# Nelarius/rayfinder

Hardware: AMD Instinct MI355X
Metric: Mrays/sec at 1920x1080 Sponza, 8 bounces; achieved HBM GB/s on traversal (higher is better)
Workload: dtype f32

## Files before the change

include/rayfinder_amd.h:

```cpp
#ifndef RAYFINDER_AMD_H
#define RAYFINDER_AMD_H

#include <stddef.h>
#include <stdint.h>

#ifdef __cplusplus
extern "C" {
#endif

#define RF_API __attribute__((visibility("default")))

typedef enum rf_status
{
    RF_OK = 0,
    RF_ERROR_INVALID_ARGUMENT = 1,
    RF_ERROR_RUNTIME = 2,
    RF_ERROR_NO_DEVICE = 3,
    RF_ERROR_OUT_OF_RANGE = 4,
} rf_status;

RF_API const char* rf_last_error_message(void);
RF_API const char* rf_version(void);

typedef struct rf_camera
// ... 92 lines not shown
{
    uint32_t iterations;
    float    sigma_color, sigma_normal, sigma_depth;
} rf_denoise_parameters;
RF_API int rf_denoise_default_parameters(rf_denoise_parameters* out);
RF_API int rf_renderer_denoise(rf_renderer* r, const rf_denoise_parameters* params);
RF_API int rf_renderer_read_denoised(rf_renderer* r, float* rgba, uint32_t* bgra8, uint32_t* sample_count);
RF_API int rf_denoise_images(int32_t device_ordinal, uint32_t width, uint32_t height, uint32_t samples, const float* color_sum4, const float* albedo_coverage4,
                             const float* normal_depth4, const rf_denoise_parameters* params, float exposure, float* out_rgba, uint32_t* out_bgra8);
RF_API int rf_denoise_tiles(int32_t device_ordinal, uint32_t width, uint32_t height, const uint32_t* tile_samples, const float* color_sum4,
                            const float* albedo_coverage4, const float* normal_depth4, const rf_denoise_parameters* params, float exposure, float* out_rgba,
                            uint32_t* out_bgra8);

RF_API int rf_renderer_set_direct(rf_renderer* r, int enabled);
RF_API int rf_renderer_read_direct(rf_renderer* r, float* direct_sum4, uint32_t* direct_sample_count);
RF_API int rf_denoise_split_default_parameters(rf_denoise_parameters* direct, rf_denoise_parameters* indirect);
RF_API int rf_renderer_denoise_split(rf_renderer* r, const rf_denoise_parameters* direct, const rf_denoise_parameters* indirect);
RF_API int rf_denoise_split_images(int32_t device_ordinal, uint32_t width, uint32_t height, uint32_t samples, const float* color_sum4, const float* direct_sum4,
                                   const float* albedo_coverage4, const float* normal_depth4, const rf_denoise_parameters* direct, const rf_denoise_parameters* indirect,
                                   float exposure, float* out_rgba, uint32_t* out_bgra8);

typedef struct rf_noise_estimate
{
    double   mean_error;
    float    max_error;
    uint32_t worst_tile, samples;
    uint64_t pixels, nonfinite_pixels;
} rf_noise_estimate;
RF_API int rf_renderer_set_moments(rf_renderer* r, int enabled);
RF_API int rf_renderer_read_moments(rf_renderer* r, float* sumsq4, uint32_t* moment_sample_count);
RF_API int rf_renderer_noise_estimate(rf_renderer* r, rf_noise_estimate* out, float* error_map, float* tile_sum, float* tile_max);
RF_API int rf_noise_estimate_images(int32_t device_ordinal, uint32_t width, uint32_t height, uint32_t samples, const float* color_sum4, const float* sumsq4,
                                    rf_noise_estimate* out, float* error_map, float* tile_sum, float* tile_max);
RF_API int rf_renderer_render_until(rf_renderer* r, float target_mean_error, uint32_t check_every, uint32_t max_frames, uint32_t* frames_rendered,
                                    rf_noise_estimate* last);

#define RF_BUCKETS_TILE_COUNTS 0x100u
#define RF_BUCKETS_SHARD_TILE_COUNTS 0x400u
RF_API int rf_renderer_set_buckets(rf_renderer* r, uint32_t K);
RF_API int rf_renderer_read_buckets(rf_renderer* r, float* buckets, uint32_t* K, uint32_t* bucket_sample_count);
RF_API int rf_renderer_robust_mean(rf_renderer* r);
RF_API int rf_renderer_read_robust_mean(rf_renderer* r, float* rgba, uint32_t* bgra8, uint8_t* trim, uint32_t* sample_count);
RF_API int rf_robust_mean_images(int32_t device_ordinal, uint32_t width, uint32_t height, uint32_t K, uint32_t samples, const float* buckets, float exposure,
                                 float* out_rgba, uint32_t* out_bgra8, uint8_t* out_trim);
RF_API int rf_robust_mean_tiles(int32_t device_ordinal, uint32_t width, uint32_t height, uint32_t K, const uint32_t* tile_samples, const float* buckets, float exposure,
                                float* out_rgba, uint32_t* out_bgra8, uint8_t* out_trim);
RF_API int rf_renderer_denoise_robust(rf_renderer* r, const rf_denoise_parameters* params);

typedef struct rf_adaptive_parameters
{
    float    target_tile_error;
    uint32_t check_every, min_samples, max_samples;
} rf_adaptive_parameters;
typedef struct rf_adaptive_result
{
    uint32_t          estimate_passes, tiles, stopped_tiles, min_tile_samples, max_tile_samples, reserved;
    uint64_t          pixel_samples;
    rf_noise_estimate last;
} rf_adaptive_result;
RF_API int rf_renderer_render_adaptive(rf_renderer* r, const rf_adaptive_parameters* params, rf_adaptive_result* result);
RF_API int rf_renderer_read_tile_samples(rf_renderer* r, uint32_t* tile_samples, uint32_t* num_tiles);
RF_API int rf_renderer_read_mean(rf_renderer* r, float* rgba);
RF_API int rf_noise_estimate_tiles(int32_t device_ordinal, uint32_t width, uint32_t height, const uint32_t* tile_samples, const float* color_sum4, const float* sumsq4,
                                   rf_noise_estimate* out, float* error_map, float* tile_sum, float* tile_max);

RF_API int rf_renderer_render_deferred(rf_renderer* r, uint32_t num_frames);
RF_API int rf_renderer_reset_deferred(rf_renderer* r);
RF_API int rf_renderer_read_deferred(rf_renderer* r, float* sample_rgb, float* accumulation_rgb, uint32_t* bgra8, uint32_t* frame_count);

RF_API int rf_renderer_set_counting(rf_renderer* r, int enabled);
RF_API int rf_renderer_set_timing(rf_renderer* r, int enabled);
RF_API int rf_renderer_set_option(rf_renderer* r, const char* name, int64_t value);
RF_API int rf_renderer_reset_stats(rf_renderer* r);
RF_API int rf_renderer_get_stats(rf_renderer* r, rf_stats* out);
RF_API int rf_renderer_get_bounce_stats(rf_renderer* r, uint32_t capacity, uint64_t* closest_rays, uint64_t* shadow_rays,
                                        double* ms_closest, double* ms_shadow, uint32_t* num_bounces);

RF_API int rf_renderer_set_tile_shard(rf_renderer* r, uint32_t rank, uint32_t world_size);
RF_API int rf_renderer_shard_tiles(rf_renderer* r, uint32_t* tile_ids , uint32_t* num_tiles);
RF_API int rf_renderer_accumulation_device_buffer(rf_renderer* r, void** device_ptr, uint64_t* bytes);
RF_API int rf_renderer_bind_accumulation_buffer(rf_renderer* r, void* device_ptr, uint64_t bytes);

RF_API int rf_device_count(int32_t* count_out);
typedef struct rf_comm rf_comm;
#define RF_COMM_ID_BYTES 128
#define RF_GATHER_LOOPBACK 1u
#define RF_GATHER_AOVS    2u
#define RF_GATHER_MOMENTS 4u
#define RF_GATHER_TILE_COUNTS 8u
#define RF_GATHER_ROBUST_MEAN 16u
RF_API int  rf_comm_unique_id(uint8_t id_out[RF_COMM_ID_BYTES]);
RF_API int  rf_comm_create(const uint8_t id[RF_COMM_ID_BYTES], uint32_t rank, uint32_t world_size, int32_t device_ordinal, rf_comm** out);
RF_API void rf_comm_destroy(rf_comm* c);
RF_API int  rf_renderer_gather_frame(rf_renderer* r, rf_comm* c, uint32_t root, uint32_t flags, void** image_device_out );
RF_API int  rf_renderer_tonemap_device_image(rf_renderer* r, const void* image_device, uint64_t num_pixels, uint32_t samples, uint32_t* dst_bgra8);
RF_API int  rf_comm_read_frame(rf_comm* c, rf_renderer* r, float* dst);
RF_API int  rf_comm_gathered_planes(const rf_comm* c, uint32_t* flags_out, uint32_t* width, uint32_t* height, uint32_t* samples);
RF_API int  rf_comm_read_plane(rf_comm* c, rf_renderer* r, uint32_t plane , float* dst);
RF_API int  rf_comm_plane_device(rf_comm* c, uint32_t plane, void** device_ptr);
RF_API int  rf_comm_denoise(rf_comm* c, rf_renderer* r, const rf_denoise_parameters* params);
RF_API int  rf_comm_read_denoised(rf_comm* c, rf_renderer* r, float* rgba, uint32_t* bgra8, uint32_t* sample_count);
RF_API int  rf_comm_noise_estimate(rf_comm* c, rf_renderer* r, rf_noise_estimate* out, float* error_map, float* tile_sum, float* tile_max);
typedef struct rf_comm_adaptive_result
{
    rf_adaptive_result rank;
    uint32_t frame_leading_samples;
    uint32_t frame_min_tile_samples;
    uint64_t max_rank_pixel_samples;
} rf_comm_adaptive_result;
RF_API int  rf_comm_render_adaptive(rf_comm* c, rf_renderer* r, const rf_adaptive_parameters* params, rf_comm_adaptive_result* result);
RF_API int  rf_comm_read_tile_samples(rf_comm* c, uint32_t* tile_samples , uint32_t* num_tiles);
RF_API int  rf_comm_read_mean(rf_comm* c, rf_renderer* r, float* rgba);
RF_API int  rf_comm_read_robust_mean(rf_comm* c, rf_renderer* r, float* rgba, uint32_t* bgra8, uint8_t* trim, uint32_t* K, uint32_t* sample_count);
RF_API int  rf_comm_denoise_robust(rf_comm* c, rf_renderer* r, const rf_denoise_parameters* params);
RF_API int  rf_comm_all_reduce_max(rf_comm* c, rf_renderer* r , double* value);
RF_API int  rf_comm_info(const rf_comm* c, uint32_t* rccl_ranks, uint32_t* rccl_rank, int32_t* device_ordinal);
RF_API int  rf_comm_transport(const rf_comm* c, uint32_t* local_out);
RF_API int  rf_comm_last_exchange_ms(rf_comm* c, double* ms_out);
RF_API int  rf_renderer_memory_info(const rf_renderer* r, uint64_t* path_state_bytes, uint64_t* paths_allocated, uint64_t* max_paths_per_batch, uint64_t* scene_bytes);
enum { RF_LAYOUT_BINARY = 0, RF_LAYOUT_COMPACT = 1, RF_LAYOUT_HOT = 2, RF_LAYOUT_QUAD = 3, RF_LAYOUT_QUAD_HALF = 4, RF_LAYOUT_QUAD_LOCAL = 5, RF_LAYOUT_OCT = 6,
       RF_LAYOUT_SCALAR = 7, RF_LAYOUT_PACKET = 8 };
typedef struct rf_layout_info
{
    uint32_t closest_layout[16];
    uint32_t shadow_layout[16];
    uint32_t shadow_cached[16];
    uint32_t occluder_hint_levels;
    uint32_t shadow_first_look_from_bounce;
    uint32_t dense_leaf_min;
    uint32_t legacy_layouts_compiled;
    float    quad_half_area_ratio;
    float    reserved;
    uint64_t tree_bytes;
} rf_layout_info;
RF_API int  rf_renderer_layout_info(const rf_renderer* r, rf_layout_info* out);
typedef struct rf_launch_plan
{
    uint32_t num_samples, num_bounces;
    uint32_t sample_perm;
    uint32_t dense_raygen;
    uint32_t const_origin;
    uint32_t primary_layout;
    uint32_t occluder_grid, occluder_scale_bits, occluder_mask;
    uint32_t runs;
    uint32_t tile_list;
    uint32_t accumulate_kernel;
    uint32_t accumulate_pixels, aov_pixels, moment_pixels;
    uint32_t raygen_count_word;
    uint32_t closest_kernel, closest_layout, closest_counting, closest_nearest, closest_dense, closest_refill_min, closest_chunk, closest_leaf_vote, closest_flags, closest_extra_lds;
    uint32_t closest_count_word, closest_cursor_word;
    uint32_t shade_sorted, shade_aov, shade_flags, shade_sort_scale, shade_grid_cap;
    uint32_t shadow_kernel, shadow_layout, shadow_counting, shadow_nearest, shadow_dense, shadow_refill_min, shadow_chunk, shadow_leaf_vote, shadow_flags, shadow_extra_lds;
    uint32_t shadow_count_word, shadow_cursor_word;
    uint32_t shadow_cached;
    uint32_t shadow_first_look;
    uint32_t shadow_self;
    uint32_t shadow_source;
    uint32_t look_flags, look_count_word, look_list_word;
} rf_launch_plan;
RF_API int  rf_renderer_launch_plan(const rf_renderer* r, uint32_t bounce, uint32_t num_samples, rf_launch_plan* out);
typedef struct rf_gather_op
{
    uint32_t is_send, peer, offset_tiles, count_tiles;
} rf_gather_op;
RF_API int rf_gather_plan(uint32_t width, uint32_t height, uint32_t world_size, uint32_t rank, uint32_t root, uint32_t flags, rf_gather_op* ops, uint32_t* num_ops);
RF_API int rf_gather_plan_counts(uint32_t width, uint32_t height, uint32_t world_size, uint32_t rank, uint32_t root, uint32_t flags, rf_gather_op* ops, uint32_t* num_ops);
// ... 97 lines not shown
```

rayfinder_amd/__init__.py:

```python
import ctypes as C

import numpy as np

from . import _ffi
from ._ffi import RayfinderError, check, lib

NODE_DTYPE = np.dtype([("min", "<f4", 3), ("pad0", "<f4"), ("max", "<f4", 3), ("pad1", "<f4"),
                       ("trianglesOffset", "<u4"), ("secondChildOffset", "<u4"),
                       ("triangleCount", "<u4"), ("splitAxis", "<u4")])
TILE = 32


def _ptr(a):
    return None if a is None else a.ctypes.data_as(C.c_void_p)


def _f32(a):
    return np.ascontiguousarray(a, dtype=np.float32)


def version():
    return lib.rf_version().decode()


# ... 257 lines not shown

    def scene(self):
        v = self.view()
        textures = (_ffi.Texture * max(int(v.num_textures), 1))()
        sc = _ffi.Scene()
        check(lib.rf_pt_format_scene(self._h, C.byref(sc), textures))
        sc._keepalive = (textures, self)
        return sc


def scene_from_arrays(nodes, positions48, attrs80, textures):
    nodes = np.ascontiguousarray(nodes)
    pos = _f32(positions48).reshape(-1, 12)
    att = np.ascontiguousarray(attrs80, dtype=np.float32).reshape(-1, 20)
    keep = [np.ascontiguousarray(px, np.uint32) for px, _, _ in textures]
    arr = (_ffi.Texture * max(len(textures), 1))()
    for i, (px, w, h) in enumerate(textures):
        arr[i] = _ffi.Texture(keep[i].ctypes.data, w, h)
    sc = _ffi.Scene(nodes.ctypes.data, nodes.shape[0], pos.ctypes.data, att.ctypes.data, pos.shape[0], arr, len(textures))
    sc._keepalive = (nodes, pos, att, keep, arr)
    return sc


RF_GATHER_LOOPBACK = 1
RF_GATHER_AOVS = 2
RF_GATHER_MOMENTS = 4
RF_GATHER_TILE_COUNTS = 8
RF_GATHER_ROBUST_MEAN = 16


def _gather_flags(loopback=False, aovs=False, moments=False, tile_counts=False, robust_mean=False):
    return ((RF_GATHER_LOOPBACK if loopback else 0) | (RF_GATHER_AOVS if aovs else 0) | (RF_GATHER_MOMENTS if moments else 0) | (RF_GATHER_TILE_COUNTS if tile_counts else 0)
            | (RF_GATHER_ROBUST_MEAN if robust_mean else 0))


class _GatheredPlanes(dict):

    def __missing__(self, key):
        if key in ("tile_counts", "robust_mean"):
            return False
        raise KeyError(key)


def gather_layout(width, height, world_size):
    n = ((width + 31) // 32) * ((height + 31) // 32)
    first = np.zeros(world_size + 1, np.uint32); slot = np.zeros(n, np.uint32); owner = np.zeros(n, np.uint32)
    check(lib.rf_gather_layout(width, height, world_size, _ptr(first), _ptr(slot), _ptr(owner)))
    return first, slot, owner


def gather_plan(width, height, world_size, rank, root=0, loopback=False):
    n = C.c_uint32(0)
    flags = RF_GATHER_LOOPBACK if loopback else 0
    check(lib.rf_gather_plan(width, height, world_size, rank, root, flags, None, C.byref(n)))
    ops = np.zeros((n.value, 4), np.uint32)
    check(lib.rf_gather_plan(width, height, world_size, rank, root, flags, _ptr(ops), C.byref(n)))
    return ops


def gather_plan_planes(width, height, world_size, rank, root=0, loopback=False, aovs=False, moments=False, robust_mean=False):
    n = C.c_uint32(0)
    flags = _gather_flags(loopback, aovs, moments, robust_mean=robust_mean)
    check(lib.rf_gather_plan_planes(width, height, world_size, rank, root, flags, None, C.byref(n)))
    ops = np.zeros((n.value, 5), np.uint32)
    check(lib.rf_gather_plan_planes(width, height, world_size, rank, root, flags, _ptr(ops), C.byref(n)))
    return ops


def gather_plan_counts(width, height, world_size, rank, root=0, loopback=False):
    n = C.c_uint32(0)
    flags = RF_GATHER_LOOPBACK if loopback else 0
    check(lib.rf_gather_plan_counts(width, height, world_size, rank, root, flags, None, C.byref(n)))
    ops = np.zeros((n.value, 4), np.uint32)
    check(lib.rf_gather_plan_counts(width, height, world_size, rank, root, flags, _ptr(ops), C.byref(n)))
    return ops


def device_count():
    n = C.c_int32(0)
    check(lib.rf_device_count(C.byref(n)))
    return n.value


def comm_unique_id():
    buf = np.zeros(128, np.uint8)
    check(lib.rf_comm_unique_id(_ptr(buf)))
    return buf.tobytes()


class TileComm:

    def __init__(self, unique_id, rank, world_size, device_ordinal=0):
        buf = np.frombuffer(bytes(unique_id), np.uint8).copy()
        assert buf.size == 128
        self._h = C.c_void_p()
        self.rank, self.world_size = rank, world_size
        check(lib.rf_comm_create(_ptr(buf), rank, world_size, device_ordinal, C.byref(self._h)))

    def close(self):
        if getattr(self, "_h", None) and lib is not None:
            lib.rf_comm_destroy(self._h)
            self._h = None

    def __del__(self):
        self.close()

    def info(self):
        n, r, d = C.c_uint32(0), C.c_uint32(0), C.c_int32(0)
        check(lib.rf_comm_info(self._h, C.byref(n), C.byref(r), C.byref(d)))
        return dict(rccl_ranks=n.value, rccl_rank=r.value, device=d.value)

    def local_transport(self):
        v = C.c_uint32(0)
        check(lib.rf_comm_transport(self._h, C.byref(v)))
        return bool(v.value)

    def last_exchange_ms(self):
        v = C.c_double(-1.0)
        check(lib.rf_comm_last_exchange_ms(self._h, C.byref(v)))
        return v.value

    def read_frame(self, renderer, width, height):
        img = np.zeros((height, width, 4), np.float32)
        check(lib.rf_comm_read_frame(self._h, renderer._h, _ptr(img)))
        return img

    def all_reduce_max(self, value, renderer=None):
        v = C.c_double(value)
        check(lib.rf_comm_all_reduce_max(self._h, renderer._h if renderer is not None else None, C.byref(v)))
        return v.value

    def gathered_planes(self):
        f, w, h, n = C.c_uint32(0), C.c_uint32(0), C.c_uint32(0), C.c_uint32(0)
        check(lib.rf_comm_gathered_planes(self._h, C.byref(f), C.byref(w), C.byref(h), C.byref(n)))
        out = _GatheredPlanes(aovs=bool(f.value & RF_GATHER_AOVS), moments=bool(f.value & RF_GATHER_MOMENTS), width=w.value, height=h.value, samples=n.value)
        if f.value & RF_GATHER_TILE_COUNTS:
            out["tile_counts"] = True
        if f.value & RF_GATHER_ROBUST_MEAN:
            out["robust_mean"] = True
        return out

    def read_plane(self, renderer, plane):
        g = self.gathered_planes()
        img = np.zeros((g["height"], g["width"], 4), np.float32)
        check(lib.rf_comm_read_plane(self._h, renderer._h, plane, _ptr(img)))
        return img

    def denoise(self, renderer, params=None):
        check(lib.rf_comm_denoise(self._h, renderer._h, C.byref(_denoise_parameters(dict(params or {})))))

    def read_denoised(self, renderer):
        g = self.gathered_planes()
        rgba = np.zeros((g["height"], g["width"], 4), np.float32)
        bgra = np.zeros((g["height"], g["width"]), np.uint32)
        n = C.c_uint32(0)
        check(lib.rf_comm_read_denoised(self._h, renderer._h, _ptr(rgba), _ptr(bgra), C.byref(n)))
        return rgba[..., :3], bgra, n.value

    def noise_estimate(self, renderer, maps=True):
        g = self.gathered_planes()
        est = _ffi.NoiseEstimate()
        emap = tsum = tmax = None
        if maps:
            emap = np.zeros((g["height"], g["width"]), np.float32)
            tsum = np.zeros(_noise_tiles(g["width"], g["height"]), np.float32); tmax = np.zeros_like(tsum)
        check(lib.rf_comm_noise_estimate(self._h, renderer._h, C.byref(est), _ptr(emap) if maps else None, _ptr(tsum) if maps else None, _ptr(tmax) if maps else None))
# ... 459 lines not shown
```

rayfinder_amd/_ffi.py:

```python
import ctypes as C
import os

_HERE = os.path.dirname(os.path.abspath(__file__))
LIB_PATH = os.environ.get("RAYFINDER_AMD_LIB") or os.path.join(_HERE, "librayfinder_amd.so")
if os.environ.get("RAYFINDER_AMD_LIB"):
    import sys
    print(f"[rayfinder_amd] RAYFINDER_AMD_LIB overrides the packaged library: loading {LIB_PATH}", file=sys.stderr, flush=True)

if not os.path.exists(LIB_PATH):
    raise ImportError(
        f"{LIB_PATH} is missing: build the HIP extension first (make -C rayfinder_amd/csrc). "
        "rayfinder_amd has no CPU fallback.")

try:
    import torch
except ImportError:
    pass
lib = C.CDLL(LIB_PATH)

RF_OK = 0
RF_ERROR_INVALID_ARGUMENT = 1
RF_ERROR_RUNTIME = 2
RF_ERROR_NO_DEVICE = 3
RF_ERROR_OUT_OF_RANGE = 4
# ... 63 lines not shown
                ("ms_raygen", C.c_double), ("ms_closest", C.c_double), ("ms_shade", C.c_double), ("ms_shadow", C.c_double),
                ("ms_accumulate", C.c_double),
                ("launches_raygen", C.c_uint32), ("launches_closest", C.c_uint32), ("launches_shade", C.c_uint32),
                ("launches_shadow", C.c_uint32), ("launches_accumulate", C.c_uint32), ("batches_traced", C.c_uint32),
                ("closest_record_fetches", C.c_uint64), ("shadow_record_fetches", C.c_uint64),
                ("abandoned_rays", C.c_uint64), ("scalar_redo_rays", C.c_uint64), ("shadow_rays_hint_answered", C.c_uint64), ("shadow_rays_self_answered", C.c_uint64)]

    def as_dict(self):
        return {k: getattr(self, k) for k, _ in self._fields_ if not k.startswith("reserved")}


class PtFormatView(C.Structure):
    _fields_ = [("bvh_nodes", C.c_void_p), ("num_bvh_nodes", C.c_uint64),
                ("bvh_position_attributes", C.c_void_p), ("num_bvh_position_attributes", C.c_uint64),
                ("triangle_position_attributes", C.c_void_p), ("num_triangle_position_attributes", C.c_uint64),
                ("triangle_vertex_attributes", C.c_void_p), ("num_triangle_vertex_attributes", C.c_uint64),
                ("vertex_positions", C.c_void_p), ("num_vertex_positions", C.c_uint64),
                ("vertex_normals", C.c_void_p), ("num_vertex_normals", C.c_uint64),
                ("vertex_tex_coords", C.c_void_p), ("num_vertex_tex_coords", C.c_uint64),
                ("vertex_indices", C.c_void_p), ("num_vertex_indices", C.c_uint64),
                ("model_vertex_positions", C.c_void_p), ("num_model_vertex_positions", C.c_uint64),
                ("model_vertex_normals", C.c_void_p), ("num_model_vertex_normals", C.c_uint64),
                ("model_vertex_tex_coords", C.c_void_p), ("num_model_vertex_tex_coords", C.c_uint64),
                ("model_vertex_indices", C.c_void_p), ("num_model_vertex_indices", C.c_uint64),
                ("model_base_color_texture_indices", C.c_void_p), ("num_model_base_color_texture_indices", C.c_uint64),
                ("num_textures", C.c_uint64)]


SIGNATURES = {
    "rf_last_error_message": (C.c_char_p, []),
    "rf_version": (C.c_char_p, []),
    "rf_renderer_create": (C.c_int, [C.POINTER(RendererDescriptor), C.POINTER(Scene), C.POINTER(C.c_void_p)]),
    "rf_renderer_destroy": (None, [C.c_void_p]),
    "rf_renderer_set_render_parameters": (C.c_int, [C.c_void_p, C.POINTER(RenderParameters)]),
    "rf_renderer_render": (C.c_int, [C.c_void_p, C.c_uint32]),
    "rf_renderer_synchronize": (C.c_int, [C.c_void_p]),
    "rf_renderer_average_renderpass_duration_ms": (C.c_float, [C.c_void_p]),
    "rf_renderer_render_progress_percentage": (C.c_float, [C.c_void_p]),
    "rf_renderer_read_accumulation": (C.c_int, [C.c_void_p, C.c_void_p, C.POINTER(C.c_uint32)]),
    "rf_renderer_read_tonemapped": (C.c_int, [C.c_void_p, C.c_void_p]),
    "rf_renderer_set_aovs": (C.c_int, [C.c_void_p, C.c_uint32]),
    "rf_renderer_read_aovs": (C.c_int, [C.c_void_p, C.c_void_p, C.c_void_p, C.POINTER(C.c_uint32)]),
    "rf_denoise_default_parameters": (C.c_int, [C.c_void_p]),
    "rf_renderer_denoise": (C.c_int, [C.c_void_p, C.c_void_p]),
    "rf_renderer_read_denoised": (C.c_int, [C.c_void_p, C.c_void_p, C.c_void_p, C.POINTER(C.c_uint32)]),
    "rf_denoise_images": (C.c_int, [C.c_int32, C.c_uint32, C.c_uint32, C.c_uint32, C.c_void_p, C.c_void_p, C.c_void_p, C.c_void_p, C.c_float, C.c_void_p,
                                    C.c_void_p]),
    "rf_denoise_tiles": (C.c_int, [C.c_int32, C.c_uint32, C.c_uint32, C.c_void_p, C.c_void_p, C.c_void_p, C.c_void_p, C.c_void_p, C.c_float, C.c_void_p, C.c_void_p]),
    "rf_renderer_set_direct": (C.c_int, [C.c_void_p, C.c_int]),
    "rf_renderer_read_direct": (C.c_int, [C.c_void_p, C.c_void_p, C.POINTER(C.c_uint32)]),
    "rf_denoise_split_default_parameters": (C.c_int, [C.c_void_p, C.c_void_p]),
    "rf_renderer_denoise_split": (C.c_int, [C.c_void_p, C.c_void_p, C.c_void_p]),
    "rf_denoise_split_images": (C.c_int, [C.c_int32, C.c_uint32, C.c_uint32, C.c_uint32, C.c_void_p, C.c_void_p, C.c_void_p, C.c_void_p, C.c_void_p, C.c_void_p, C.c_float,
                                          C.c_void_p, C.c_void_p]),
    "rf_renderer_set_moments": (C.c_int, [C.c_void_p, C.c_int]),
    "rf_renderer_read_moments": (C.c_int, [C.c_void_p, C.c_void_p, C.POINTER(C.c_uint32)]),
    "rf_renderer_set_buckets": (C.c_int, [C.c_void_p, C.c_uint32]),
    "rf_renderer_read_buckets": (C.c_int, [C.c_void_p, C.c_void_p, C.POINTER(C.c_uint32), C.POINTER(C.c_uint32)]),
    "rf_renderer_robust_mean": (C.c_int, [C.c_void_p]),
    "rf_renderer_read_robust_mean": (C.c_int, [C.c_void_p, C.c_void_p, C.c_void_p, C.c_void_p, C.POINTER(C.c_uint32)]),
    "rf_robust_mean_images": (C.c_int, [C.c_int32, C.c_uint32, C.c_uint32, C.c_uint32, C.c_uint32, C.c_void_p, C.c_float, C.c_void_p, C.c_void_p, C.c_void_p]),
    "rf_robust_mean_tiles": (C.c_int, [C.c_int32, C.c_uint32, C.c_uint32, C.c_uint32, C.c_void_p, C.c_void_p, C.c_float, C.c_void_p, C.c_void_p, C.c_void_p]),
    "rf_renderer_denoise_robust": (C.c_int, [C.c_void_p, C.c_void_p]),
    "rf_renderer_noise_estimate": (C.c_int, [C.c_void_p, C.c_void_p, C.c_void_p, C.c_void_p, C.c_void_p]),
    "rf_noise_estimate_images": (C.c_int, [C.c_int32, C.c_uint32, C.c_uint32, C.c_uint32, C.c_void_p, C.c_void_p, C.c_void_p, C.c_void_p, C.c_void_p, C.c_void_p]),
    "rf_renderer_render_until": (C.c_int, [C.c_void_p, C.c_float, C.c_uint32, C.c_uint32, C.POINTER(C.c_uint32), C.c_void_p]),
    "rf_renderer_render_adaptive": (C.c_int, [C.c_void_p, C.c_void_p, C.c_void_p]),
    "rf_renderer_read_tile_samples": (C.c_int, [C.c_void_p, C.c_void_p, C.POINTER(C.c_uint32)]),
    "rf_renderer_read_mean": (C.c_int, [C.c_void_p, C.c_void_p]),
    "rf_noise_estimate_tiles": (C.c_int, [C.c_int32, C.c_uint32, C.c_uint32, C.c_void_p, C.c_void_p, C.c_void_p, C.c_void_p, C.c_void_p, C.c_void_p, C.c_void_p]),
    "rf_renderer_render_deferred": (C.c_int, [C.c_void_p, C.c_uint32]),
    "rf_renderer_reset_deferred": (C.c_int, [C.c_void_p]),
    "rf_renderer_read_deferred": (C.c_int, [C.c_void_p, C.c_void_p, C.c_void_p, C.c_void_p, C.POINTER(C.c_uint32)]),
    "rf_renderer_set_counting": (C.c_int, [C.c_void_p, C.c_int]),
    "rf_renderer_set_timing": (C.c_int, [C.c_void_p, C.c_int]),
    "rf_renderer_set_option": (C.c_int, [C.c_void_p, C.c_char_p, C.c_int64]),
    "rf_renderer_reset_stats": (C.c_int, [C.c_void_p]),
    "rf_renderer_get_stats": (C.c_int, [C.c_void_p, C.POINTER(Stats)]),
    "rf_renderer_set_tile_shard": (C.c_int, [C.c_void_p, C.c_uint32, C.c_uint32]),
    "rf_renderer_shard_tiles": (C.c_int, [C.c_void_p, C.c_void_p, C.POINTER(C.c_uint32)]),
    "rf_renderer_accumulation_device_buffer": (C.c_int, [C.c_void_p, C.POINTER(C.c_void_p), C.POINTER(C.c_uint64)]),
    "rf_renderer_bind_accumulation_buffer": (C.c_int, [C.c_void_p, C.c_void_p, C.c_uint64]),
    "rf_device_count": (C.c_int, [C.POINTER(C.c_int32)]),
    "rf_comm_unique_id": (C.c_int, [C.c_void_p]),
    "rf_comm_create": (C.c_int, [C.c_void_p, C.c_uint32, C.c_uint32, C.c_int32, C.POINTER(C.c_void_p)]),
    "rf_comm_destroy": (None, [C.c_void_p]),
    "rf_renderer_gather_frame": (C.c_int, [C.c_void_p, C.c_void_p, C.c_uint32, C.c_uint32, C.POINTER(C.c_void_p)]),
    "rf_renderer_tonemap_device_image": (C.c_int, [C.c_void_p, C.c_void_p, C.c_uint64, C.c_uint32, C.c_void_p]),
    "rf_comm_read_frame": (C.c_int, [C.c_void_p, C.c_void_p, C.c_void_p]),
    "rf_comm_all_reduce_max": (C.c_int, [C.c_void_p, C.c_void_p, C.POINTER(C.c_double)]),
    "rf_comm_gathered_planes": (C.c_int, [C.c_void_p] + [C.POINTER(C.c_uint32)] * 4),
    "rf_comm_read_plane": (C.c_int, [C.c_void_p, C.c_void_p, C.c_uint32, C.c_void_p]),
    "rf_comm_plane_device": (C.c_int, [C.c_void_p, C.c_uint32, C.POINTER(C.c_void_p)]),
    "rf_comm_denoise": (C.c_int, [C.c_void_p, C.c_void_p, C.c_void_p]),
    "rf_comm_read_denoised": (C.c_int, [C.c_void_p, C.c_void_p, C.c_void_p, C.c_void_p, C.POINTER(C.c_uint32)]),
    "rf_comm_noise_estimate": (C.c_int, [C.c_void_p] * 6),
    "rf_comm_render_adaptive": (C.c_int, [C.c_void_p, C.c_void_p, C.c_void_p, C.c_void_p]),
    "rf_comm_read_tile_samples": (C.c_int, [C.c_void_p, C.c_void_p, C.POINTER(C.c_uint32)]),
    "rf_comm_read_mean": (C.c_int, [C.c_void_p, C.c_void_p, C.c_void_p]),
    "rf_comm_read_robust_mean": (C.c_int, [C.c_void_p, C.c_void_p, C.c_void_p, C.c_void_p, C.c_void_p, C.POINTER(C.c_uint32), C.POINTER(C.c_uint32)]),
    "rf_comm_denoise_robust": (C.c_int, [C.c_void_p, C.c_void_p, C.c_void_p]),
    "rf_comm_info": (C.c_int, [C.c_void_p, C.POINTER(C.c_uint32), C.POINTER(C.c_uint32), C.POINTER(C.c_int32)]),
    "rf_renderer_layout_info": (C.c_int, [C.c_void_p, C.c_void_p]),
    "rf_renderer_launch_plan": (C.c_int, [C.c_void_p, C.c_uint32, C.c_uint32, C.c_void_p]),
    "rf_renderer_memory_info": (C.c_int, [C.c_void_p] + [C.POINTER(C.c_uint64)] * 4),
    "rf_gather_plan": (C.c_int, [C.c_uint32] * 6 + [C.c_void_p, C.POINTER(C.c_uint32)]),
    "rf_gather_plan_planes": (C.c_int, [C.c_uint32] * 6 + [C.c_void_p, C.POINTER(C.c_uint32)]),
    "rf_gather_plan_counts": (C.c_int, [C.c_uint32] * 6 + [C.c_void_p, C.POINTER(C.c_uint32)]),
    "rf_gather_layout": (C.c_int, [C.c_uint32, C.c_uint32, C.c_uint32, C.c_void_p, C.c_void_p, C.c_void_p]),
    "rf_tiles_for_rank": (C.c_int, [C.c_uint32, C.c_uint32, C.c_uint32, C.c_uint32, C.c_void_p, C.POINTER(C.c_uint32)]),
    "rf_untile": (C.c_int, [C.c_void_p, C.c_void_p, C.c_uint32, C.c_uint32, C.c_uint32, C.c_void_p]),
    "rf_renderer_trace_primary_stats": (C.c_int, [C.c_void_p, C.POINTER(Camera), C.c_uint32, C.c_uint32, C.c_void_p, C.c_void_p, C.c_void_p, C.c_void_p]),
    "rf_renderer_get_bounce_stats": (C.c_int, [C.c_void_p, C.c_uint32] + [C.c_void_p] * 5),
    "rf_renderer_intersect_rays": (C.c_int, [C.c_void_p, C.c_void_p, C.c_uint64, C.c_float] + [C.c_void_p] * 6),
    "rf_renderer_occluded_rays": (C.c_int, [C.c_void_p, C.c_void_p, C.c_uint64, C.c_float, C.c_void_p]),
    "rf_intersect_bvh": (C.c_int, [C.c_void_p, C.c_void_p, C.c_uint64, C.c_void_p, C.c_uint32, C.c_uint64, C.c_float, C.c_void_p, C.c_void_p, C.POINTER(C.c_int)]),
    "rf_intersect_bvh_batch": (C.c_int, [C.c_void_p, C.c_uint64, C.c_void_p, C.c_uint64, C.c_void_p, C.c_uint32, C.c_uint64, C.c_float, C.c_uint32, C.c_void_p, C.c_void_p, C.c_void_p]),
    "rf_bvh_visualizer_pass": (C.c_int, [C.POINTER(Camera), C.c_uint32, C.c_uint32, C.c_uint32, C.c_uint32, C.c_void_p, C.c_uint64, C.c_void_p, C.c_uint32, C.c_uint64, C.c_uint32,
                                         C.c_void_p, C.c_void_p, C.c_void_p, C.c_void_p]),
    "rf_build_bvh": (C.c_int, [C.c_void_p, C.c_uint64, C.c_void_p, C.POINTER(C.c_uint64), C.c_void_p, C.POINTER(C.c_int32)]),
    "rf_comm_last_exchange_ms": (C.c_int, [C.c_void_p, C.POINTER(C.c_double)]),
    "rf_comm_transport": (C.c_int, [C.c_void_p, C.POINTER(C.c_uint32)]),
    "rf_check_wide_layouts": (C.c_int, [C.c_void_p, C.c_uint64, C.POINTER(C.c_uint32)]),
    "rf_wide_layout_stats": (C.c_int, [C.c_void_p, C.c_uint64, C.POINTER(C.c_uint32), C.POINTER(C.c_float)]),
    "rf_build_bvh_gpu": (C.c_int, [C.c_void_p, C.c_uint64, C.c_void_p, C.c_void_p, C.c_void_p, C.c_void_p, C.c_int32, C.c_void_p]),
    "rf_create_camera": (C.c_int, [C.c_void_p, C.c_void_p, C.c_float, C.c_float, C.c_float, C.c_float, C.POINTER(Camera)]),
    "rf_fly_camera": (C.c_int, [C.c_void_p] + [C.c_float] * 6 + [C.POINTER(Camera)]),
    "rf_bvh_visualizer_camera": (C.c_int, [C.c_void_p, C.c_float, C.POINTER(Camera)]),
    "rf_sky_state_new": (C.c_int, [C.c_float, C.c_float, C.c_void_p, C.c_void_p]),
    "rf_sky_state_radiance": (C.c_float, [C.c_void_p, C.c_float, C.c_float, C.c_int]),
    "rf_aligned_sky_state": (C.c_int, [C.POINTER(Sky), C.c_void_p]),
    "rf_texture_from_memory": (C.c_int, [C.c_void_p, C.c_uint64, C.c_void_p, C.c_void_p, C.c_void_p]),
    "rf_pt_format_set_bvh_builder": (C.c_int, [C.c_int32]),
    "rf_pt_format_from_gltf": (C.c_int, [C.c_char_p, C.POINTER(C.c_void_p)]),
    "rf_pt_format_load": (C.c_int, [C.c_char_p, C.POINTER(C.c_void_p)]),
    "rf_pt_format_deserialize": (C.c_int, [C.c_void_p, C.c_uint64, C.POINTER(C.c_void_p)]),
    "rf_pt_format_save": (C.c_int, [C.c_void_p, C.c_char_p]),
    "rf_pt_format_serialize": (C.c_int, [C.c_void_p, C.c_void_p, C.POINTER(C.c_uint64)]),
    "rf_pt_format_from_triangles": (C.c_int, [C.c_void_p, C.c_void_p, C.c_void_p, C.c_void_p, C.c_uint64, C.POINTER(Texture), C.c_uint64, C.POINTER(C.c_void_p)]),
    "rf_pt_format_view_get": (C.c_int, [C.c_void_p, C.POINTER(PtFormatView)]),
    "rf_pt_format_texture": (C.c_int, [C.c_void_p, C.c_uint64, C.POINTER(Texture)]),
    "rf_pt_format_destroy": (None, [C.c_void_p]),
    "rf_pt_format_scene": (C.c_int, [C.c_void_p, C.POINTER(Scene), C.POINTER(Texture)]),
}

for _name, (_res, _args) in SIGNATURES.items():
    _fn = getattr(lib, _name)
    _fn.restype = _res
    _fn.argtypes = _args


class RayfinderError(RuntimeError):
    def __init__(self, status, message):
        super().__init__(message)
        self.status = status


def check(status):
    if status != RF_OK:
        raise RayfinderError(status, lib.rf_last_error_message().decode("utf-8", "replace"))
```

rayfinder_amd/csrc/rf_c_api.cpp:

```cpp
#include "../../include/rayfinder_amd.h"

#include "rf_bvh.hpp"
#include "rf_bvh_gpu.hpp"
#include "rf_camera.hpp"
#include "rf_comm.hpp"
#include "rf_gltf.hpp"
#include "rf_pt_format.hpp"
#include "rf_query.hpp"
#include "rf_renderer.hpp"
#include "rf_sky.hpp"

#include <cstring>
#include <exception>
#include <new>
#include <stdexcept>
#include <string>
#include <vector>

static_assert(sizeof(rf_camera) == sizeof(rf::Camera));
static_assert(RF_AOV_FIRST_HIT == rf::Renderer::kAovFirstHit);
static_assert(RF_AOV_TILE_COUNTS == rf::Renderer::kAovTileCounts);
static_assert(RF_BUCKETS_TILE_COUNTS == rf::Renderer::kBucketsTileCounts);
static_assert(RF_BUCKETS_SHARD_TILE_COUNTS == rf::Renderer::kBucketsShardTileCounts);

// ... 616 lines not shown

int rf_renderer_get_stats(rf_renderer* r, rf_stats* out)
{
    return guarded([&] {
        require(r && out, "null argument");
        const rf::RenderStats s = r->impl->stats();
        std::memset(out, 0, sizeof *out);
        out->primary_rays = s.primaryRays;
        out->closest_rays = s.closestRays;
        out->shadow_rays = s.shadowRays;
        out->closest_node_visits = s.closestNodeVisits;
        out->closest_triangle_tests = s.closestTriangleTests;
        out->shadow_node_visits = s.shadowNodeVisits;
        out->shadow_triangle_tests = s.shadowTriangleTests;
        out->paths = s.paths;
        out->stack_high_water = s.stackHighWater;
        out->batch_samples_used = s.batchSamplesUsed;
        out->batches_traced = s.batchesTraced;
        out->ms_raygen = s.msRaygen;
        out->ms_closest = s.msClosest;
        out->ms_shade = s.msShade;
        out->ms_shadow = s.msShadow;
        out->ms_accumulate = s.msAccumulate;
        out->launches_raygen = s.launchesRaygen;
        out->launches_closest = s.launchesClosest;
        out->launches_shade = s.launchesShade;
        out->launches_shadow = s.launchesShadow;
        out->launches_accumulate = s.launchesAccumulate;
        out->closest_record_fetches = s.closestRecordFetches;
        out->shadow_record_fetches = s.shadowRecordFetches;
        out->abandoned_rays = s.abandonedRays;
        out->scalar_redo_rays = s.scalarRedoRays;
        out->shadow_rays_hint_answered = s.shadowRaysHintAnswered;
        out->shadow_rays_self_answered = s.shadowRaysSelfAnswered;
        return RF_OK;
    });
}

int rf_renderer_set_tile_shard(rf_renderer* r, uint32_t rank, uint32_t world_size)
{
    return guarded([&] {
        require(r, "null argument");
        require(world_size > 0 && rank < world_size, "invalid rank / world size");
        r->impl->setTileShard(rank, world_size);
        return RF_OK;
    });
}

int rf_renderer_shard_tiles(rf_renderer* r, uint32_t* tile_ids, uint32_t* num_tiles)
{
    return guarded([&] {
        require(r && num_tiles, "null argument");
        const auto tiles = r->impl->shardTiles();
        *num_tiles = static_cast<uint32_t>(tiles.size());
        if (tile_ids) std::memcpy(tile_ids, tiles.data(), tiles.size() * sizeof(uint32_t));
        return RF_OK;
    });
}

int rf_renderer_accumulation_device_buffer(rf_renderer* r, void** device_ptr, uint64_t* bytes)
{
    return guarded([&] {
        require(r && device_ptr && bytes, "null argument");
        *device_ptr = r->impl->accumulationDevicePointer();
        *bytes = r->impl->accumulationBytes();
        return RF_OK;
    });
}

int rf_renderer_bind_accumulation_buffer(rf_renderer* r, void* device_ptr, uint64_t bytes)
{
    return guarded([&] {
        require(r, "null argument");
        r->impl->bindAccumulationBuffer(device_ptr, bytes);
        return RF_OK;
    });
}

int rf_device_count(int32_t* count_out)
{
    return guarded([&] {
        require(count_out, "null argument");
        *count_out = rf::deviceCount();
        return RF_OK;
    });
}

int rf_comm_unique_id(uint8_t id_out[RF_COMM_ID_BYTES])
{
    return guarded([&] {
        require(id_out, "null argument");
        rf::TileComm::uniqueId(id_out);
        return RF_OK;
    });
}

int rf_comm_create(const uint8_t id[RF_COMM_ID_BYTES], uint32_t rank, uint32_t world_size, int32_t device_ordinal, rf_comm** out)
{
    return guarded([&] {
        require(id && out, "null argument");
        require(world_size > 0 && rank < world_size, "invalid rank / world size");
        auto h = std::make_unique<rf_comm>();
        h->impl = std::make_unique<rf::TileComm>(id, rank, world_size, device_ordinal);
        *out = h.release();
        return RF_OK;
    });
}

void rf_comm_destroy(rf_comm* c) { delete c; }

int rf_renderer_gather_frame(rf_renderer* r, rf_comm* c, uint32_t root, uint32_t flags, void** image_device_out)
{
    return guarded([&] {
        require(r && c, "null argument");
        const void* image = rf::gatherFrame(*r->impl, *c->impl, root, flags);
        if (image_device_out) *image_device_out = const_cast<void*>(image);
        return RF_OK;
    });
}

int rf_renderer_tonemap_device_image(rf_renderer* r, const void* image_device, uint64_t num_pixels, uint32_t samples, uint32_t* dst)
{
    return guarded([&] {
        require(r && image_device && dst, "null argument");
        require(samples > 0, "samples must be > 0");
        r->impl->tonemapDeviceImage(image_device, num_pixels, samples, dst);
        return RF_OK;
    });
}

int rf_comm_read_frame(rf_comm* c, rf_renderer* r, float* dst)
{
    return guarded([&] {
        require(c && r && dst, "null argument");
        c->impl->readFrame(dst, r->impl->streamHandle());
        return RF_OK;
    });
}

int rf_comm_gathered_planes(const rf_comm* c, uint32_t* flags_out, uint32_t* width, uint32_t* height, uint32_t* samples)
{
    return guarded([&] {
        require(c, "null argument");
        uint32_t mask = 0, w = 0, h = 0, n = 0;
        c->impl->gatheredPlanes(mask, w, h, n);
        if (flags_out) *flags_out = ((mask & rf::kPlaneMaskAovs) == rf::kPlaneMaskAovs ? RF_GATHER_AOVS : 0u) | ((mask & rf::kPlaneMaskMoments) ? RF_GATHER_MOMENTS : 0u) |
                                        ((mask & rf::kGatherMaskTileCounts) ? RF_GATHER_TILE_COUNTS : 0u) | ((mask & rf::kPlaneMaskRobustMean) ? RF_GATHER_ROBUST_MEAN : 0u);
        if (width) *width = w;
        if (height) *height = h;
        if (samples) *samples = n;
        return RF_OK;
    });
}

int rf_comm_read_plane(rf_comm* c, rf_renderer* r, uint32_t plane, float* dst)
{
    return guarded([&] {
        require(c && r && dst, "null argument");
        c->impl->readPlane(plane, dst, r->impl->streamHandle());
        return RF_OK;
    });
}

int rf_comm_plane_device(rf_comm* c, uint32_t plane, void** device_ptr)
{
    return guarded([&] {
// ... 645 lines not shown
```

rayfinder_amd/csrc/rf_device.hpp:

```cpp
#pragma once

#include "rf_types.hpp"

#include <hip/hip_runtime.h>

namespace rf
{
constexpr int      kBlock = 256;
constexpr int      kLdsStack = 24;
constexpr int      kSpillStack = 72;
constexpr uint32_t kMiss = 0xFFFFFFFFu;
constexpr uint32_t kLeafAxis = 3u;
constexpr uint32_t kTriStride = 4u;

struct DeviceScene
{
    const float4*            nodes;
    const float4*            triangles;
    const float4*            attributes;
    const float4*            shadeRecords;
    const TextureDescriptor* textureDescriptors;
    const uint32_t*          texels;
    uint64_t                 numTexels;
    const uint8_t*           blueNoise;
    const float*             albedoLut;
};

#if defined(__HIPCC__)
struct RayPrep
{
    Vec3     origin;
    Vec3     direction;
    Vec3     invDir;
    uint32_t negX, negY, negZ;
};

__device__ __forceinline__ RayPrep prepareRay(Vec3 o, Vec3 d)
{
    RayPrep r;
    r.origin = o;
    r.direction = d;
    r.invDir = vec3(1.0f / d.x, 1.0f / d.y, 1.0f / d.z);
    r.negX = r.invDir.x < 0.0f;
    r.negY = r.invDir.y < 0.0f;
    r.negZ = r.invDir.z < 0.0f;
    return r;
}

__device__ __forceinline__ bool slabTest(const RayPrep& r, float4 lo, float4 hi, float rayTMax)
{
    float       tmin = ((r.negX ? hi.x : lo.x) - r.origin.x) * r.invDir.x;
    float       tmax = ((r.negX ? lo.x : hi.x) - r.origin.x) * r.invDir.x;
    const float tymin = ((r.negY ? hi.y : lo.y) - r.origin.y) * r.invDir.y;
    const float tymax = ((r.negY ? lo.y : hi.y) - r.origin.y) * r.invDir.y;
    if ((tmin > tymax) || (tymin > tmax)) return false;
    tmin = maxf(tymin, tmin);
    tmax = minf(tymax, tmax);
    const float tzmin = ((r.negZ ? hi.z : lo.z) - r.origin.z) * r.invDir.z;
    const float tzmax = ((r.negZ ? lo.z : hi.z) - r.origin.z) * r.invDir.z;
    if ((tmin > tzmax) || (tzmin > tmax)) return false;
    tmin = maxf(tzmin, tmin);
    tmax = minf(tzmax, tmax);
    return (tmin < rayTMax) && (tmax > 0.0f);
}

__device__ __forceinline__ Vec3 offsetRay(Vec3 p, Vec3 n)
{
    constexpr float kOrigin = 1.0f / 32.0f;
    constexpr float kFloatScale = 1.0f / 65536.0f;
    constexpr float kIntScale = 256.0f;
    const int       ox = static_cast<int>(kIntScale * n.x);
    const int       oy = static_cast<int>(kIntScale * n.y);
    const int       oz = static_cast<int>(kIntScale * n.z);
    const Vec3      shifted = vec3(__int_as_float(__float_as_int(p.x) + (p.x < 0 ? -ox : ox)),
                                   __int_as_float(__float_as_int(p.y) + (p.y < 0 ? -oy : oy)),
                                   __int_as_float(__float_as_int(p.z) + (p.z < 0 ? -oz : oz)));
    return vec3(fabsf(p.x) < kOrigin ? p.x + kFloatScale * n.x : shifted.x,
                fabsf(p.y) < kOrigin ? p.y + kFloatScale * n.y : shifted.y,
                fabsf(p.z) < kOrigin ? p.z + kFloatScale * n.z : shifted.z);
}

struct TriangleHit
{
    float t, u, v;
};

__device__ __forceinline__ bool
intersectTriangle(Vec3 origin, Vec3 direction, Vec3 p0, Vec3 p1, Vec3 p2, float rayTMax, TriangleHit& hit)
{
    constexpr float kEpsilon = 0.00001f;
    const Vec3      e1 = p1 - p0;
    const Vec3      e2 = p2 - p0;
    const Vec3      h = cross(direction, e2);
    const float     det = dot(e1, h);
    if (det > -kEpsilon && det < kEpsilon) return false;
    const float invDet = 1.0f / det;
    const Vec3  s = origin - p0;
    const float u = invDet * dot(s, h);
    if (u < 0.0f || u > 1.0f) return false;
    const Vec3  q = cross(s, e1);
    const float v = invDet * dot(direction, q);
    if (v < 0.0f || u + v > 1.0f) return false;
    const float t = invDet * dot(e2, q);
    if (t > kEpsilon && t < rayTMax)
    {
        hit.t = t;
        hit.u = u;
        hit.v = v;
        return true;
    }
    return false;
}
__device__ __forceinline__ bool
intersectTriangle(const RayPrep& r, Vec3 p0, Vec3 p1, Vec3 p2, float rayTMax, TriangleHit& hit)
{
    return intersectTriangle(r.origin, r.direction, p0, p1, p2, rayTMax, hit);
}

struct ClosestHit
{
    uint32_t triangle;
    float    t, u, v;
    Vec3     p;
};

struct TraversalCounters
{
    uint32_t nodesVisited = 0;
    uint32_t triangleTests = 0;
    uint32_t stackHigh = 0;
    uint32_t abandoned = 0;
};

template<bool ANY_HIT, bool COUNT, int LDS = kLdsStack>
__device__ __forceinline__ bool traverse(const DeviceScene& scene, Vec3 origin, Vec3 direction, float rayTMax,
                                         uint32_t* ldsStackLane, ClosestHit& out, TraversalCounters& counters)
{
    const RayPrep ray = prepareRay(origin, direction);
    constexpr int kSpill = kLdsStack + kSpillStack - LDS;
    uint32_t      spill[kSpill];
    int           stackSize = 0;
    uint32_t      current = 0;
    bool          found = false;
    out.triangle = kMiss;

    for (;;)
    {
        const float4 lo = scene.nodes[2 * current];
        const float4 hi = scene.nodes[2 * current + 1];
        if (COUNT) ++counters.nodesVisited;
        bool advance = false;
        if (slabTest(ray, lo, hi, rayTMax))
        {
            const uint32_t link = __float_as_uint(lo.w);
            const uint32_t meta = __float_as_uint(hi.w);
            const uint32_t axis = meta & 3u;
            if (axis == kLeafAxis)
            {
                const uint32_t count = meta >> 2;
                for (uint32_t i = 0; i < count; ++i)
                {
                    const uint32_t tri = link + i;
                    const float4   a = scene.triangles[kTriStride * tri];
                    const float4   b = scene.triangles[kTriStride * tri + 1];
                    const float4   c = scene.triangles[kTriStride * tri + 2];
                    if (COUNT) ++counters.triangleTests;
                    TriangleHit th;
                    const Vec3  p0 = vec3(a.x, a.y, a.z), p1 = vec3(b.x, b.y, b.z), p2 = vec3(c.x, c.y, c.z);
                    if (intersectTriangle(ray, p0, p1, p2, rayTMax, th))
                    {
                        if (ANY_HIT) return true;
                        rayTMax = th.t;
                        found = true;
                        const Vec3 e1 = p1 - p0, e2 = p2 - p0;
                        const Vec3 p = p0 + th.u * e1 + th.v * e2;
                        const Vec3 n = normalize(cross(e1, e2));
                        out.p = offsetRay(p, n);
                        out.t = th.t;
                        out.u = th.u;
                        out.v = th.v;
                        out.triangle = tri;
                    }
                }
            }
            else
            {
                const uint32_t neg = axis == 0 ? ray.negX : (axis == 1 ? ray.negY : ray.negZ);
                const uint32_t deferred = neg ? current + 1 : link;
                current = neg ? link : current + 1;
                if (LDS > 0 && stackSize < LDS) ldsStackLane[stackSize * kBlock] = deferred;
                else if (stackSize - LDS < kSpill) spill[stackSize - LDS] = deferred;
                else
                {
                    counters.abandoned = 1;
                    break;
                }
                ++stackSize;
                if (COUNT) counters.stackHigh = max(counters.stackHigh, static_cast<uint32_t>(stackSize));
                advance = true;
            }
        }
        if (!advance)
        {
            if (stackSize == 0) break;
            --stackSize;
            if constexpr (LDS > 0)
            {
                current = ldsStackLane[min(stackSize, LDS - 1) * kBlock];
                asm volatile("" : "+v"(current));
                if (stackSize >= LDS) current = spill[stackSize - LDS];
            }
            else
            {
                current = spill[stackSize];
            }
        }
    }
    return found;
}

__device__ __forceinline__ double dExp(double x)
{
    if (x != x) return x;
    if (x > 709.0) return __builtin_inf();
    if (x < -745.0) return 0.0;
    const double k = __builtin_rint(x * 1.44269504088896338700e+00);
    double       r = __builtin_fma(-k, 6.93147180369123816490e-01, x);
    r = __builtin_fma(-k, 1.90821492927058770002e-10, r);
    double p = 1.6059043836821613e-10;
    p = __builtin_fma(p, r, 2.08767569878681e-09);
    p = __builtin_fma(p, r, 2.505210838544172e-08);
    p = __builtin_fma(p, r, 2.755731922398589e-07);
    p = __builtin_fma(p, r, 2.7557319223985893e-06);
    p = __builtin_fma(p, r, 2.48015873015873e-05);
    p = __builtin_fma(p, r, 0.0001984126984126984);
    p = __builtin_fma(p, r, 0.001388888888888889);
    p = __builtin_fma(p, r, 0.008333333333333333);
    p = __builtin_fma(p, r, 0.041666666666666664);
    p = __builtin_fma(p, r, 0.16666666666666666);
    p = __builtin_fma(p, r, 0.5);
    p = __builtin_fma(p, r, 1.0);
    p = __builtin_fma(p, r, 1.0);
    return __builtin_ldexp(p, static_cast<int>(k));
}
__device__ __forceinline__ double dReduce(double x, long long& quadrant)
{
    const double k = __builtin_rint(x * 6.36619772367581382433e-01);
    double       r = __builtin_fma(-k, 1.57079632673412561417e+00, x);
    r = __builtin_fma(-k, 6.07710050650619224932e-11, r);
    r = __builtin_fma(-k, 2.02226624879595063154e-21, r);
    quadrant = static_cast<long long>(k);
    return r;
}
__device__ __forceinline__ double dSinCosKernel(double r, bool cosine)
{
    const double z = r * r;
    const double c5 = cosine ? -1.13596475577881948265e-11 : 1.58969099521155010221e-10, c4 = cosine ? 2.08757232129817482790e-09 : -2.50507602534068634195e-08;
// ... 137 lines not shown
```

rayfinder_amd/csrc/rf_kernels.hpp:

```cpp
#pragma once

#include "rf_renderer.hpp"

#include "rf_bvh.hpp"
#include "rf_camera.hpp"
#include "rf_data.hpp"
#include "rf_device.hpp"
#include "rf_hip_host.hpp"
#include "rf_wide.hpp"

#include <hip/hip_runtime.h>

#include <algorithm>
#include <cfloat>
#include <cmath>
#include <cstdio>
#include <cstdlib>
#include <cstring>
#include <functional>
#include <stdexcept>
#include <string>
#include <type_traits>

namespace rf
// ... 157 lines not shown

constexpr int kItems = 4;

template<int ITEMS>
__device__ __forceinline__ void blockAppend(const bool (&keep)[ITEMS], const uint32_t (&slot)[ITEMS], uint32_t* queue, uint32_t* count, uint32_t* sScratch,
                                            uint32_t (*position)[ITEMS] = nullptr, const uint32_t (*second)[ITEMS] = nullptr, uint32_t* queue2 = nullptr)
{
    const uint32_t lane = __lane_id(), wave = threadIdx.x >> 6;
    uint32_t       offs[ITEMS];
    uint32_t       waveTotal = 0;
#pragma unroll
    for (int k = 0; k < ITEMS; ++k)
    {
        const unsigned long long mask = __ballot(keep[k]);
        offs[k] = waveTotal + __popcll(mask & ((1ull << lane) - 1ull));
        waveTotal += __popcll(mask);
    }
    if (lane == 0) sScratch[wave] = waveTotal;
    __syncthreads();
    if (threadIdx.x == 0)
    {
        const uint32_t total = sScratch[0] + sScratch[1] + sScratch[2] + sScratch[3];
        sScratch[4] = total ? atomicAdd(count, total) : 0u;
    }
    __syncthreads();
    uint32_t base = sScratch[4];
    for (uint32_t w = 0; w < wave; ++w) base += sScratch[w];
#pragma unroll
    for (int k = 0; k < ITEMS; ++k)
    {
        if (keep[k]) queue[base + offs[k]] = slot[k];
        if (second != nullptr && keep[k]) queue2[base + offs[k]] = (*second)[k];
        if (position) (*position)[k] = base + offs[k];
    }
    __syncthreads();
}

__device__ __forceinline__ unsigned long long waveSum(unsigned long long v)
{
    for (int off = 32; off > 0; off >>= 1) v += __shfl_down(v, off);
    return v;
}
__device__ __forceinline__ uint32_t waveMax(uint32_t v)
{
    for (int off = 32; off > 0; off >>= 1) v = max(v, static_cast<uint32_t>(__shfl_down(v, off)));
    return v;
}

template<bool MAX>
__device__ __forceinline__ uint32_t waveScanInclusive(uint32_t x)
{
    const auto step = [&](auto ctrl, auto rowMask) {
        const uint32_t y = static_cast<uint32_t>(__builtin_amdgcn_update_dpp(0, static_cast<int>(x), decltype(ctrl)::value, decltype(rowMask)::value, 0xF, true));
        x = MAX ? max(x, y) : x + y;
    };
    step(std::integral_constant<int, 0x111>{}, std::integral_constant<int, 0xF>{});
    step(std::integral_constant<int, 0x112>{}, std::integral_constant<int, 0xF>{});
    step(std::integral_constant<int, 0x114>{}, std::integral_constant<int, 0xF>{});
    step(std::integral_constant<int, 0x118>{}, std::integral_constant<int, 0xF>{});
    step(std::integral_constant<int, 0x142>{}, std::integral_constant<int, 0xA>{});
    step(std::integral_constant<int, 0x143>{}, std::integral_constant<int, 0xC>{});
    return x;
}
__device__ __forceinline__ uint32_t laneGather(uint32_t value, uint32_t srcLane) { return static_cast<uint32_t>(__builtin_amdgcn_ds_bpermute(static_cast<int>(srcLane << 2), static_cast<int>(value))); }
__device__ __forceinline__ float    laneGather(float value, uint32_t srcLane) { return __uint_as_float(laneGather(__float_as_uint(value), srcLane)); }

__device__ __forceinline__ uint32_t sampleKey(uint32_t firstFrame, uint32_t spp, uint32_t k)
{
    const uint32_t n = (firstFrame + k) % spp;
    const float    rx = wFract(0.7548776662466927f * static_cast<float>(n)), ry = wFract(0.5698402909980532f * static_cast<float>(n));
    uint32_t       x = static_cast<uint32_t>(rx * 65536.0f) & 0xFFFFu, y = static_cast<uint32_t>(ry * 65536.0f) & 0xFFFFu;
    const auto     spread = [](uint32_t v) {
        v = (v | (v << 8)) & 0x00FF00FFu;
        v = (v | (v << 4)) & 0x0F0F0F0Fu;
        v = (v | (v << 2)) & 0x33333333u;
        v = (v | (v << 1)) & 0x55555555u;
        return v;
    };
    return spread(x) | (spread(y) << 1);
}

__device__ __forceinline__ Vec3 hitPoint(const DeviceScene& scene, uint32_t tri, float u, float v)
{
    const Vec3 p0 = load3(scene.triangles + kTriStride * tri), p1 = load3(scene.triangles + kTriStride * tri + 1),
               p2 = load3(scene.triangles + kTriStride * tri + 2);
    const Vec3   e1 = p1 - p0, e2 = p2 - p0;
    const Vec3   p = p0 + u * e1 + v * e2;
    return offsetRay(p, normalize(cross(e1, e2)));
}

struct SunBasis
{
    Vec3 u, v;
};

__device__ __forceinline__ Vec3 sunSample(const SkyStateGpu& sky, const SunBasis& basis, float nx, float cosPhi, float sinPhi)
{
    const float cosThetaMax = __uint_as_float(kSolarCosThetaMaxBits);
    const float cosTheta = 1.0f - nx * (1.0f - cosThetaMax);
    const float sinTheta = rf_sqrt(1.0f - cosTheta * cosTheta);
    const Vec3  local = vec3(cosPhi * sinTheta, sinPhi * sinTheta, cosTheta);
    const Vec3  sun = vec3(sky.sunDirection[0], sky.sunDirection[1], sky.sunDirection[2]);
    return basisTimes(basis.u, basis.v, sun, local);
}

constexpr uint32_t kShadeLastBounce = 1u, kShadeFirstBounce = 2u;
constexpr uint32_t kShadeSelfShadow = 4u;
constexpr uint32_t kLookFirstBounce = 1u, kLookNoRayCount = 2u;


constexpr uint32_t kSortBins = 256;

constexpr uint32_t kChunk = 128;
constexpr uint32_t kShards = 16;
constexpr uint32_t kLineWords = 16;
constexpr uint32_t kRefillMin = 40;
constexpr uint32_t kLeafVote = 20;

constexpr int kLayoutBinary = 0, kLayoutCompact = 1, kLayoutHot = 2, kLayoutQuad = 3, kLayoutQuadHalf = 4, kLayoutQuadLocal = 5, kLayoutOct = 6, kLayoutScalar = 7, kLayoutPacket = 8;
constexpr uint32_t kFlagShadowDirFromStream = 1u;
constexpr uint32_t kFlagUniformTri = 8u;
constexpr uint32_t kFlagUniformFetch = 4u;
constexpr uint32_t kFlagFirstBounce = 2u;
constexpr uint32_t kFlagOccluderCache = 16u;
constexpr uint32_t kFlagOccluderNoTry = 32u;
constexpr uint32_t kFlagNoRayCount = 64u;
constexpr uint32_t kFlagConstOrigin = 128u;
constexpr uint32_t kFlagDenseLeafShift = 8u;
#if defined(RF_EXP_OCC_SLOTS)
constexpr int kOccSlots = RF_EXP_OCC_SLOTS;
#else
constexpr int kOccSlots = 4;
#endif
static_assert(kOccSlots == 1 || kOccSlots == 2 || kOccSlots == 4, "one aligned load per cell");
constexpr uint32_t kNodeIdle = 0xFFFFFFFFu;
constexpr uint32_t kNodeDone = 0xFFFFFFFEu;


using SamplePermutationKernel = void (*)(uint32_t firstFrame, uint32_t spp, uint32_t numSamples, uint32_t* perm, uint32_t* inv);
using RaygenKernel = void (*)(FrameParams fp, DeviceScene scene, const uint32_t* tileIds, PathStreams ps, uint32_t* queue, uint32_t* queueCount, DeviceCounters* counters);
using TraceClosestKernel = void (*)(DeviceScene scene, PathStreams ps, const uint32_t* queue, const uint32_t* queueCount, DeviceCounters* counters);
using ShadeKernel = void (*)(DeviceScene scene, SkyStateGpu sky, SunBasis sunBasis, PathStreams ps, const uint32_t* queue, const uint32_t* queueCount, uint32_t* hitQueue, uint32_t* hitCount, uint32_t* missQueue, uint32_t* missSlots, uint32_t* missCount, uint32_t* shadowList, uint32_t* shadowListCount, uint32_t bounceFlags, uint32_t sortScale, float4* aov);
using SkyKernel = void (*)(SkyStateGpu sky, PathStreams ps, const uint32_t* missSlots, const uint32_t* missQueue, const uint32_t* missCount, uint32_t firstBounce);
using TraceShadowKernel = void (*)(DeviceScene scene, SkyStateGpu sky, SunBasis sunBasis, PathStreams ps, const uint32_t* queue, const uint32_t* queueCount, DeviceCounters* counters, uint32_t firstBounce);
using TraceWideKernel = void (*)(DeviceScene scene, WideScene wide, SkyStateGpu sky, SunBasis sunBasis, PathStreams ps, const uint32_t* queue, const uint32_t* queueCount, uint32_t* cursor, DeviceCounters* counters, uint32_t refillMin, uint32_t leafVote, uint32_t chunkMax, float tMax, uint32_t flags);
using ShadowFirstLookKernel = void (*)(DeviceScene scene, WideScene wide, SkyStateGpu sky, SunBasis sunBasis, PathStreams ps, const uint32_t* queue, const uint32_t* inList, const uint32_t* inCount, uint32_t* list, uint32_t* listCount, DeviceCounters* counters, float tMax, uint32_t flags);
using TracePacketKernel = void (*)(DeviceScene scene, WideScene wide, SkyStateGpu sky, SunBasis sunBasis, PathStreams ps, const uint32_t* queue, const uint32_t* queueCount, DeviceCounters* counters, float tMax, uint32_t flags);
using HitPointsKernel = void (*)(DeviceScene scene, const float4* hit, P3* rayO, uint32_t n);
using BounceTotalsKernel = void (*)(const uint32_t* queueCounts, uint32_t numBounces, unsigned long long* totals, const uint32_t* listCounts, unsigned long long lookMask, unsigned long long* lookBatch, const uint32_t* shadowListCounts, unsigned long long selfMask, DeviceCounters* counters);
using TonemapKernel = void (*)(const float4* image, uint32_t n, uint32_t accumulatedSamples, float exposure, uint32_t* out);
using PrimaryStatsKernel = void (*)(DeviceScene scene, Camera cam, uint32_t width, uint32_t height, uint32_t* nodesVisited, uint8_t* hitOut, float* tOut, uint32_t* triTests, DeviceCounters* counters);
using IntersectRaysKernel = void (*)(DeviceScene scene, const float* rays, uint64_t n, float tMax, uint32_t* triOut, float* tOut, float* uvOut, float* pOut, uint32_t* nvOut, uint32_t* ttOut, DeviceCounters* counters);
using OccludedRaysKernel = void (*)(DeviceScene scene, const float* rays, uint64_t n, float tMax, float* visOut, DeviceCounters* counters);
using DeferredLightingKernel = void (*)(DeviceScene scene, SkyStateGpu sky, SunBasis sunBasis, Camera cam, uint32_t width, uint32_t height, uint32_t frameCount, float jitterX, float jitterY, float exposure, float* sampleBuffer, float* accumulationBuffer, uint32_t* bgraOut, DeviceCounters* counters);

TraceWideKernel       traceWideKernel(bool anyHit, bool count, bool nearestFirst, int compact, bool denseLeaves);
TraceClosestKernel    traceClosestKernel(bool count);
TraceShadowKernel     traceShadowKernel(bool count);
ShadowFirstLookKernel shadowFirstLookKernel();
TracePacketKernel     tracePacketKernel(bool anyHit);
HitPointsKernel       hitPointsKernel();
PrimaryStatsKernel    primaryStatsKernel();
IntersectRaysKernel   intersectRaysKernel();
OccludedRaysKernel    occludedRaysKernel();
SamplePermutationKernel samplePermutationKernel();
RaygenKernel            raygenKernel(bool f32Transcendentals);
ShadeKernel             shadeKernel(bool sorted, bool aov = false);
SkyKernel               skyKernel(bool f32Transcendentals);
BounceTotalsKernel      bounceTotalsKernel();
TonemapKernel           tonemapKernel();
DeferredLightingKernel  deferredLightingKernel();
}
using namespace kern;
}
```

rayfinder_amd/csrc/rf_renderer.hip:

```cpp
#include "rayfinder_amd.h"
#include "rf_denoise.hpp"
#include "rf_kernels.hpp"
#include "rf_noise.hpp"
#include "rf_robust.hpp"
#include "rf_sums.hpp"

#include <map>

#include <algorithm>
#include <cfloat>
#include <cmath>
#include <cstdio>
#include <cstdlib>
#include <cstring>
#include <functional>
#include <stdexcept>
#include <string>
#include <type_traits>

namespace rf
{
bool operator==(const RenderParameters& a, const RenderParameters& b)
{
    return a.width == b.width && a.height == b.height && std::memcmp(&a.camera, &b.camera, sizeof(Camera)) == 0 &&
// ... 1122 lines not shown
            m.wide.hot = m.wideHot.ptr;
            m.wide.own = m.wideOwn.ptr;
        }
#endif
        m.wide.quad = nullptr;
        if (wb.quadUsable && !wb.quad.empty())
        {
            m.wideQuad.upload(wb.quad.data(), wb.quad.size());
            m.wide.quad = m.wideQuad.ptr;
        }
        m.wide.quadHalf = nullptr;
        m.wide.originBound = wb.originBound;
        if (!wb.quadHalf.empty())
        {
            m.wideQuadHalf.upload(wb.quadHalf.data(), wb.quadHalf.size());
            m.wide.quadHalf = m.wideQuadHalf.ptr;
            m.optQuadHalfFromBounce = m.optQuadHalfShadowFromBounce = wb.quadHalfAreaRatio <= kQuadHalfMaxAreaRatio ? 1u : 0u;
            m.quadHalfAreaRatio = wb.quadHalfAreaRatio;
        }
        m.wide.quadLocal = nullptr;
        if (!wb.quadLocal.empty())
        {
            m.wideQuadLocal.upload(wb.quadLocal.data(), wb.quadLocal.size());
            m.wide.quadLocal = m.wideQuadLocal.ptr;
            const float ratio = wb.quadHalf.empty() ? 2.0f : wb.quadHalfAreaRatio;
            m.optQuadLocalFromBounce = m.optQuadHalfFromBounce == 0u ? 2u : 0u;
            m.optQuadLocalShadowFromBounce = ratio <= kQuadLocalShadowMaxAreaRatio ? 2u : 0u;
        }
        m.wide.oct = nullptr;
        m.treeBytes = static_cast<uint64_t>(wb.quadLocal.size()) * sizeof(uint4) + static_cast<uint64_t>(sceneView.positionAttributes.size()) * kTriStride * sizeof(float4);
        if (!wb.oct.empty())
        {
            m.wideOct.upload(wb.oct.data(), wb.oct.size());
            m.wide.oct = m.wideOct.ptr;
            m.optOctFromBounce = 0u;
        }
        m.wide.bigLeaves = m.bigLeaves.ptr;
        m.wide.rootLo = wb.rootLo;
        m.wide.rootHi = wb.rootHi;
        m.wide.rootLeaf = wb.rootLeaf;
        m.wide.numRecords = static_cast<uint32_t>(wb.nodes.size() / 4);
        m.wideUsable = wb.boxesRegular;
    }
    {
        const size_t        n = sceneView.positionAttributes.size();
        std::vector<float4> padded(kTriStride * n, make_float4(0.0f, 0.0f, 0.0f, 0.0f));
        for (size_t i = 0; i < n; ++i)
        {
            const PositionAttribute& t = sceneView.positionAttributes[i];
            padded[kTriStride * i] = make_float4(t.p0.x, t.p0.y, t.p0.z, 0.0f);
            padded[kTriStride * i + 1] = make_float4(t.p1.x, t.p1.y, t.p1.z, 0.0f);
            padded[kTriStride * i + 2] = make_float4(t.p2.x, t.p2.y, t.p2.z, 0.0f);
        }
        {
            std::vector<float> diag;
            diag.reserve(sceneView.bvhNodes.size() / 2 + 1);
            for (const BvhNode& nd : sceneView.bvhNodes)
                if (nd.triangleCount != 0)
                {
                    m.maxLeafTriangles = std::max(m.maxLeafTriangles, nd.triangleCount);
                    const float dx = nd.aabb.max.x - nd.aabb.min.x, dy = nd.aabb.max.y - nd.aabb.min.y, dz = nd.aabb.max.z - nd.aabb.min.z;
                    diag.push_back(std::sqrt(dx * dx + dy * dy + dz * dz));
                }
            const Aabb& root = sceneView.bvhNodes[0].aabb;
            const float extent = std::max({root.max.x - root.min.x, root.max.y - root.min.y, root.max.z - root.min.z});
            m.occluderHintLevels = 0;
            if (!diag.empty() && extent > 0.0f)
            {
                std::nth_element(diag.begin(), diag.begin() + diag.size() / 2, diag.end());
                const float median = diag[diag.size() / 2];
                if (median > 0.0f && std::isfinite(median) && std::isfinite(extent))
                    m.occluderHintLevels = static_cast<uint32_t>(std::clamp(static_cast<int>(std::floor(std::log2(0.003f * extent / median))) + 1, 0, 3));
            }
            if (const char* v = std::getenv("RF_OCCLUDER_HINT_LEVELS")) m.occluderHintLevels = static_cast<uint32_t>(std::clamp(std::atoi(v), 0, 8));
        }
        m.leafBoxesValid = leafBoxesIntoTriangles(sceneView.bvhNodes.data(), sceneView.bvhNodes.size(), padded.data(), n, m.occluderHintLevels, &quadIndexOfNode);
        if (!m.leafBoxesValid)
        {
            m.wide.quadHalf = m.wide.quadLocal = m.wide.oct = nullptr;
            m.wideQuadHalf.release(), m.wideQuadLocal.release(), m.wideOct.release();
            m.optQuadHalfFromBounce = m.optQuadHalfShadowFromBounce = m.optQuadLocalFromBounce = m.optQuadLocalShadowFromBounce = m.optOctFromBounce = 0u;
        }
        m.triangles.upload(padded.data(), padded.size());
    }
    {
        const size_t        n = sceneView.vertexAttributes.size();
        std::vector<float4> packed(4 * n);
        for (size_t i = 0; i < n; ++i)
        {
            const VertexAttributes& v = sceneView.vertexAttributes[i];
            packed[4 * i] = make_float4(v.n0.x, v.n0.y, v.n0.z, v.n1.x);
            packed[4 * i + 1] = make_float4(v.n1.y, v.n1.z, v.n2.x, v.n2.y);
            packed[4 * i + 2] = make_float4(v.n2.z, v.uv0.x, v.uv0.y, v.uv1.x);
            packed[4 * i + 3] = make_float4(v.uv1.y, v.uv2.x, v.uv2.y, bitsFloat(v.textureIdx));
        }
        m.attributes.upload(packed.data(), packed.size());
        std::vector<float4> rec(8 * n, make_float4(0.0f, 0.0f, 0.0f, 0.0f));
        for (size_t i = 0; i < n; ++i)
        {
            const PositionAttribute& t = sceneView.positionAttributes[i];
            rec[8 * i] = make_float4(t.p0.x, t.p0.y, t.p0.z, 0.0f);
            rec[8 * i + 1] = make_float4(t.p1.x, t.p1.y, t.p1.z, 0.0f);
            rec[8 * i + 2] = make_float4(t.p2.x, t.p2.y, t.p2.z, 0.0f);
            for (int k = 0; k < 4; ++k) rec[8 * i + 3 + k] = packed[4 * i + k];
        }
        m.selfShadowOk = treeNestedRegular;
        if (m.selfShadowOk)
        {
            std::vector<uint8_t> leaves(n, 0);
            for (const BvhNode& nd : sceneView.bvhNodes)
                for (uint32_t t = 0; t < nd.triangleCount; ++t)
                {
                    const size_t i = static_cast<size_t>(nd.trianglesOffset) + t;
                    if (i >= n) continue;
                    const bool regular = std::fabs(nd.aabb.min.x) < 1e30f && std::fabs(nd.aabb.min.y) < 1e30f && std::fabs(nd.aabb.min.z) < 1e30f && std::fabs(nd.aabb.max.x) < 1e30f &&
                                         std::fabs(nd.aabb.max.y) < 1e30f && std::fabs(nd.aabb.max.z) < 1e30f && nd.aabb.min.x <= nd.aabb.max.x && nd.aabb.min.y <= nd.aabb.max.y &&
                                         nd.aabb.min.z <= nd.aabb.max.z;
                    leaves[i] = static_cast<uint8_t>(std::min(leaves[i] + (regular ? 1 : 2), 2));
                    rec[8 * i].w = nd.aabb.min.x, rec[8 * i + 1].w = nd.aabb.min.y, rec[8 * i + 2].w = nd.aabb.min.z;
                    rec[8 * i + 7] = make_float4(nd.aabb.max.x, nd.aabb.max.y, nd.aabb.max.z, 0.0f);
                }
            for (size_t i = 0; i < n; ++i) rec[8 * i + 7].w = leaves[i] == 1 ? 1.0f : 0.0f;
        }
        m.shadeRecords.upload(rec.data(), rec.size());
    }

    {
        std::vector<TextureDescriptor> descs;
        std::vector<uint32_t>          blob;
        for (const TextureView& t : sceneView.baseColorTextures)
        {
            const uint32_t offset = static_cast<uint32_t>(blob.size());
            const size_t   n = static_cast<size_t>(t.width) * t.height;
            blob.insert(blob.end(), t.pixels, t.pixels + n);
            descs.push_back({t.width, t.height, offset});
        }
        if (blob.size() > 0xFFFFFFFFull) throw std::runtime_error("Texture buffer size exceeds the 32-bit texel offset range.");
        if (blob.empty()) blob.push_back(0xFFFFFFFFu);
        if (descs.empty()) descs.push_back({1, 1, 0});
        m.textureDescriptors.upload(descs.data(), descs.size());
        m.texels.upload(blob.data(), blob.size());
    }
    {
        m.blueNoise.upload(blueNoiseTable(), 128 * 128 * 2);
        float lut[256];
        for (int i = 0; i < 256; ++i)
            lut[i] = static_cast<float>(std::pow(static_cast<double>(static_cast<float>(i) / 255.0f), static_cast<double>(2.2f)));
        m.albedoLut.upload(lut, 256);
    }
    m.scene.nodes = m.nodes.ptr;
    m.scene.triangles = m.triangles.ptr;
    m.scene.attributes = m.attributes.ptr;
    m.scene.shadeRecords = m.shadeRecords.ptr;
    m.scene.textureDescriptors = m.textureDescriptors.ptr;
    m.scene.texels = m.texels.ptr;
    m.scene.numTexels = m.texels.count;
    m.scene.blueNoise = m.blueNoise.ptr;
    m.scene.albedoLut = m.albedoLut.ptr;

    DeviceCounters zero{};
    m.counters.upload(&zero, 1);
    {
        const std::vector<unsigned long long> z(4 * RenderStats::kMaxBounceStats, 0ull);
        m.bounceTotals.upload(z.data(), z.size());
    }
    {
// ... 1353 lines not shown
```

rayfinder_amd/csrc/rf_renderer.hpp:

```cpp
#pragma once

#include "rf_sky.hpp"
#include "rf_types.hpp"

#include <algorithm>
#include <cstddef>
#include <cstdint>
#include <deque>
#include <memory>
#include <span>
#include <string>
#include <vector>

struct rf_launch_plan;

namespace rf
{
struct SamplingParams
{
    uint32_t numSamplesPerPixel = 128;
    uint32_t numBounces = 4;
    bool     operator==(const SamplingParams&) const = default;
};

// ... 167 lines not shown
    uint32_t aovFlags() const;
    void     readAovs(float* albedoCoverage, float* normalDepth, uint32_t* sampleCount);
    void denoise(const DenoiseParameters& params);
    void readDenoised(float* rgba, uint32_t* bgra8, uint32_t* sampleCount);
    void     setMoments(bool enabled);
    bool     momentsEnabled() const;
    void     readMoments(float* sumSq, uint32_t* sampleCount);
    void     setDirect(bool enabled);
    bool     directEnabled() const;
    void     readDirect(float* directSum, uint32_t* sampleCount);
    void denoiseSplit(const DenoiseParameters& direct, const DenoiseParameters& indirect);
    static constexpr uint32_t kBucketsTileCounts = 0x100u, kBucketsShardTileCounts = 0x400u;
    void     setBuckets(uint32_t word);
    uint32_t buckets() const;
    bool     bucketsPerTile() const;
    void     readBuckets(float* planes, uint32_t* K, uint32_t* sampleCount);
    void robustMean();
    void readRobustMean(float* rgba, uint32_t* bgra8, uint8_t* trim, uint32_t* sampleCount);
    void denoiseRobust(const DenoiseParameters& params);
    NoiseEstimate noiseEstimate(float* errorMap, float* tileSum, float* tileMax);
    uint32_t renderUntil(float targetMeanError, uint32_t checkEvery, uint32_t maxFrames, NoiseEstimate* last);
    AdaptiveResult renderAdaptive(const AdaptiveParameters& params);
    void           checkAdaptive(const AdaptiveParameters& params, bool sharded = false) const;
    AdaptiveResult renderAdaptiveFrom(const AdaptiveParameters& params, uint32_t leading, bool shardSlots);
    uint32_t       settleFrameTileSamples(uint32_t leading, uint32_t minimum, uint32_t skipFrames);
    const uint32_t* shardTileSamplesDevice();
    bool           tileSamplesUniform() const;
    void           requireUniformTileSamples(const char* what) const;
    uint32_t readTileSamples(uint32_t* tileSamples) const;
    void readMean(float* rgba);
    void*    accumulationDevicePointer() const;
    struct ShardSums
    {
        struct Channel
        {
            bool     on, coversAccumulation;
            uint32_t samples;
        };
        const void* planes[4];
        Channel     aovs, moments;
        uint32_t    accumulated;
        bool        ownsTiles;
        Channel     buckets;
        uint32_t    bucketsK;
        bool        bucketsShardTileCounts;
        uint32_t    minTileSamples;
    };
    ShardSums shardSums() const;
    const void* enqueueShardRobustMean(const uint32_t* slotCounts = nullptr);
    void     clearAccumulationIfStale();
    void     layoutInfo(uint32_t (&layouts)[48], uint32_t (&misc)[4], float& quadHalfAreaRatio, uint64_t& treeBytes) const;
    void     launchPlan(uint32_t bounce, uint32_t numSamples, ::rf_launch_plan& out) const;
    void     memoryInfo(uint64_t& pathStateBytes, uint64_t& pathsAllocated, uint64_t& maxPathsPerBatch, uint64_t& sceneBytes) const;
    uint64_t accumulationBytes() const;
    void     bindAccumulationBuffer(void* devicePtr, uint64_t bytes);
    void readTonemapped(uint32_t* dstBgra8);
    void tonemapDeviceImage(const void* imageDevice, uint64_t numPixels, uint32_t samples, uint32_t* dstBgra8Host);

    void     renderDeferred(uint32_t numFrames);
    void     resetDeferred();
    uint32_t deferredFrameCount() const;
    void readDeferred(float* sampleRgb, float* accumulationRgb, uint32_t* bgra8);

    void        setCounting(bool enabled);
    void        setOption(const std::string& name, int64_t value);
    uint32_t    numBounces() const;
    void        setTiming(bool enabled);
    void        resetStats();
    RenderStats stats();
    void        synchronize();

    void tracePrimaryStats(const Camera& camera, uint32_t width, uint32_t height, uint32_t* nodesVisitedOut,
                           uint8_t* hitOut, float* tOut, uint32_t* triangleTestsOut);
    void intersectRays(const float* rays6, uint64_t numRays, float tMax, uint32_t* triangleOut, float* tOut, float* uvOut,
                       float* pOut, uint32_t* nodesVisitedOut, uint32_t* triangleTestsOut);
    void occludedRays(const float* rays6, uint64_t numRays, float tMax, float* visibilityOut);

private:
    struct Impl;
    std::unique_ptr<Impl> mImpl;
};

uint32_t checkWideLayouts(std::span<const BvhNode> nodes, float* quadHalfAreaRatio = nullptr);
}
```

rayfinder_amd/csrc/rf_shade.hip:

```cpp
#include "rf_kernels.hpp"

namespace rf
{
namespace
{
__global__ void kSamplePermutation(uint32_t firstFrame, uint32_t spp, uint32_t numSamples, uint32_t* perm, uint32_t* inv)
{
    const uint32_t k = blockIdx.x * blockDim.x + threadIdx.x;
    if (k >= numSamples) return;
    const uint32_t mine = sampleKey(firstFrame, spp, k);
    uint32_t       rank = 0;
    for (uint32_t j = 0; j < numSamples; ++j)
    {
        const uint32_t other = sampleKey(firstFrame, spp, j);
        rank += (other < mine || (other == mine && j < k)) ? 1u : 0u;
    }
    perm[rank] = k;
    inv[k] = rank;
}

template<bool F32>
__global__ __launch_bounds__(kBlock) void kRaygen(FrameParams fp, DeviceScene scene, const uint32_t* tileIds, PathStreams ps,
                                                   uint32_t* queue, uint32_t* queueCount, DeviceCounters* counters)
{
// ... 216 lines not shown
#pragma unroll
        for (int k = 0; k < kItems; ++k) hits[k] = isHit[k] ? vec3(sIn[6 * kTile + hitTri[k]], sIn[7 * kTile + hitTri[k]], sIn[8 * kTile + hitTri[k]]) : Vec3{};
    }
    struct ShadeRecord
    {
        Vec3   p0, p1, p2;
        float4 a0, a1, a2, a3;
        Vec3   boxLo;
        float4 boxHi;
    };
    const auto fetchRecord = [&](uint32_t tri) {
        ShadeRecord   r;
        const float4* rec = scene.shadeRecords + 8 * static_cast<size_t>(tri);
#if defined(RF_EXP_SHADE_ABLATE) && RF_EXP_SHADE_ABLATE >= 3
        if constexpr (SORTED) rec = scene.shadeRecords + 8 * static_cast<size_t>(tri & 63u);
#endif
        if (selfShadow)
        {
            const float4 q0 = rec[0], q1 = rec[1], q2 = rec[2];
            r.p0 = vec3(q0.x, q0.y, q0.z), r.p1 = vec3(q1.x, q1.y, q1.z), r.p2 = vec3(q2.x, q2.y, q2.z);
            r.boxLo = vec3(q0.w, q1.w, q2.w);
            r.boxHi = rec[7];
        }
        else
        {
            r.p0 = load3(rec), r.p1 = load3(rec + 1), r.p2 = load3(rec + 2);
            r.boxLo = Vec3{}, r.boxHi = make_float4(0.0f, 0.0f, 0.0f, 0.0f);
        }
        r.a0 = rec[3], r.a1 = rec[4], r.a2 = rec[5], r.a3 = rec[6];
        return r;
    };
    const auto shade = [&](int k, float hu, float hv, float hitT, const ShadeRecord& cur, uint32_t out) -> bool {
        const uint32_t i = entryIndex(k);
        (void)i;
        Vec3 shadowOrigin;
        {
            const Vec3 p0 = cur.p0, p1 = cur.p1, p2 = cur.p2;
            const Vec3 e1 = p1 - p0, e2 = p2 - p0;
            const Vec3 hp = offsetRay(p0 + hu * e1 + hv * e2, normalize(cross(e1, e2)));
            store3nt(ps.rayO + out, hp);
            shadowOrigin = hp;
        }
        Vec3 throughput, nz;
        if constexpr (SORTED)
        {
            const uint32_t local = hitTri[k];
            throughput = vec3(sIn[local], sIn[kTile + local], sIn[2 * kTile + local]);
            nz = vec3(sIn[3 * kTile + local], sIn[4 * kTile + local], sIn[5 * kTile + local]);
        }
        else
        {
            throughput = isFirstBounce ? vec3(1.0f, 1.0f, 1.0f) : load3nt(ps.thr + i);
            nz = load3nt(ps.noise + i);
        }
        const float nx = nz.x, cosPhi = nz.y, sinPhi = nz.z;
        store3nt(ps.noiseOut + out, nz);
        const float4  a0 = cur.a0, a1 = cur.a1, a2 = cur.a2, a3 = cur.a3;
        const Vec3    n0 = vec3(a0.x, a0.y, a0.z), n1 = vec3(a0.w, a1.x, a1.y), n2 = vec3(a1.z, a1.w, a2.x);
        const float   b0 = 1.0f - hu - hv, b1 = hu, b2 = hv;
        const Vec3    n = (b0 * n0 + b1 * n1) + b2 * n2;
        const float   uvx = (b0 * a2.y + b1 * a2.w) + b2 * a3.y;
        const float   uvy = (b0 * a2.z + b1 * a3.x) + b2 * a3.z;
#if defined(RF_EXP_SHADE_ABLATE) && (RF_EXP_SHADE_ABLATE == 1 || RF_EXP_SHADE_ABLATE == 4)
        const Vec3    albedo = SORTED ? vec3(sLut[__float_as_uint(a3.w) & 255u], uvx - floorf(uvx), uvy - floorf(uvy)) : evalTexture(scene, sLut, __float_as_uint(a3.w), uvx, uvy);
#else
        const Vec3    albedo = evalTexture(scene, sLut, __float_as_uint(a3.w), uvx, uvy);
#endif
        if constexpr (AOV)
        {
            const float nn = dot(n, n);
            const Vec3  unitN = (nn != 0.0f && isfinite(nn)) ? normalize(n) : Vec3{};
            storeAov(aov, slots[k], albedo, 1.0f, unitN, hitT);
        }
        else (void)hitT, (void)aov;

        const Vec3 lightDirection = sunSample(sky, sunBasis, nx, cosPhi, sinPhi);
        const Vec3 lightIntensity = vec3(sky.solarRadiances[0], sky.solarRadiances[1], sky.solarRadiances[2]);
        const Vec3 brdf = albedo * kFrac1Pi;
        const Vec3 reflectance = brdf * dot(n, lightDirection);
        const Vec3 pend = (throughput * lightIntensity) * reflectance;
        bool       settled = false;
        if (selfShadow && cur.boxHi.w != 0.0f)
        {
            const RayPrep ray = prepareRay(shadowOrigin, lightDirection);
            if (classifyRay(ray) == kRayPlain)
            {
                const PackedRay pr = packRay(ray);
                float           bn, bf;
                bool            boxNaN;
                slabSingleBounds(pr, cur.boxLo.x, cur.boxLo.y, cur.boxLo.z, cur.boxHi.x, cur.boxHi.y, cur.boxHi.z, bn, bf, boxNaN);
                if (bn <= bf && bf > 0.0f && bn < kTMax)
                {
                    TriangleHit th;
                    settled = intersectTriangle(shadowOrigin, lightDirection, cur.p0, cur.p1, cur.p2, kTMax, th);
                }
            }
        }
        if (settled)
        {
            const Vec3 add = (pend * 0.0f) * __uint_as_float(kSolarInvPdfBits);
            const bool unchanged = !isFirstBounce && add.x == 0.0f && add.y == 0.0f && add.z == 0.0f;
            if (!unchanged)
            {
                const uint32_t slot = slots[k];
                const Vec3     radiance = (isFirstBounce ? vec3(0.0f, 0.0f, 0.0f) : load3(ps.rad + slot)) + add;
                ps.rad[slot] = make_float4(radiance.x, radiance.y, radiance.z, 0.0f);
            }
        }
        else store3nt(ps.pending + out, pend);

        if (!isLastBounce)
        {
            const float sinTheta = rf_sqrt(1.0f - nx);
            const Vec3  local = vec3(cosPhi * sinTheta, sinPhi * sinTheta, rf_sqrt(nx));
            Vec3        bu, bv;
            pixarOnb(n, bu, bv);
            const Vec3 wi = basisTimes(bu, bv, n, local);
            const Vec3 t2 = throughput * albedo;
            store3nt(ps.rayDOut + out, wi);
            store3nt(ps.thrOut + out, t2);
        }
        return !settled;
    };
    bool needShadow[kItems];
    if constexpr (kPipelined)
    {
        const uint32_t tileHits = sortedHits, base = sortedBase;
        ShadeRecord    cur{};
        if (threadIdx.x < tileHits) cur = fetchRecord(__float_as_uint(hits[0].x));
#pragma unroll
        for (int k = 0; k < kItems; ++k)
        {
            const uint32_t p = static_cast<uint32_t>(k) * kBlock + threadIdx.x, pNext = p + kBlock;
            ShadeRecord    next{};
            if (k + 1 < kItems && pNext < tileHits) next = fetchRecord(__float_as_uint(hits[k + 1 < kItems ? k + 1 : k].x));
            needShadow[k] = p < tileHits && shade(k, hits[k].y, hits[k].z, 0.0f, cur, base + p);
            cur = next;
        }
    }
    else
    {
#pragma unroll
        for (int k = 0; k < kItems; ++k) needShadow[k] = false;
#pragma unroll 1
        for (int k = 0; k < kItems; ++k)
        {
            if (!isHit[k]) continue;
            Vec3  h;
            float hitT = 0.0f;
            if constexpr (AOV)
            {
                const float4 rec = ps.hit[entryIndex(k)];
                h = vec3(rec.x, rec.y, rec.z), hitT = rec.w;
            }
            else h = load3(ps.hit + entryIndex(k));
            const bool need = shade(k, h.y, h.z, hitT, fetchRecord(__float_as_uint(h.x)), outPos[k]);
#pragma unroll
            for (int j = 0; j < kItems; ++j) needShadow[j] = j == k ? need : needShadow[j];
        }
    }
    if (selfShadow) blockAppend<kItems>(needShadow, outPos, shadowList, shadowListCount, sScratch);
    if constexpr (SORTED) __syncthreads();
  }
}

template<bool F32>
__global__ __launch_bounds__(kBlock) void kSky(SkyStateGpu sky, PathStreams ps, const uint32_t* missSlots, const uint32_t* missQueue, const uint32_t* missCount,
                                                uint32_t firstBounce)
{
    const uint32_t n = *missCount;
    const bool     first = firstBounce != 0u;
    for (uint32_t i = blockIdx.x * kBlock + threadIdx.x; i < n; i += gridDim.x * kBlock)
    {
        const uint32_t q = missQueue[i];
        const uint32_t slot = missSlots[i];
        const Vec3     v = load3(ps.rayD + q);
        const Vec3     thrIn = load3(ps.thr + q), radIn = load3(ps.rad + slot);
        const Vec3     thr = first ? vec3(1.0f, 1.0f, 1.0f) : thrIn;
        const Vec3     rad = first ? vec3(0.0f, 0.0f, 0.0f) : radIn;
        const Vec3     s = vec3(sky.sunDirection[0], sky.sunDirection[1], sky.sunDirection[2]);
        const float    theta = tAcos<F32>(v.y);
        const float    gamma = tAcos<F32>(minf(maxf(dot(v, s), -1.0f), 1.0f));
        const float cosGamma = tCos<F32>(gamma), cosTheta = fabsf(tCos<F32>(theta));
        const Vec3  dome = vec3(skyRadiance<F32>(sky, cosTheta, gamma, cosGamma, 0), skyRadiance<F32>(sky, cosTheta, gamma, cosGamma, 1), skyRadiance<F32>(sky, cosTheta, gamma, cosGamma, 2));
        const Vec3  radiance = rad + thr * dome;
        ps.rad[slot] = make_float4(radiance.x, radiance.y, radiance.z, 0.0f);
    }
}

__global__ void kBounceTotals(const uint32_t* queueCounts, uint32_t numBounces, unsigned long long* totals, const uint32_t* listCounts, unsigned long long lookMask, unsigned long long* lookBatch,
                              const uint32_t* shadowListCounts, unsigned long long selfMask, DeviceCounters* counters)
{
    const uint32_t b = threadIdx.x;
    if (b >= numBounces) return;
    const uint32_t k = min(b, RenderStats::kMaxBounceStats - 1);
    atomicAdd(&totals[k], static_cast<unsigned long long>(queueCounts[kLineWords * b]));
    atomicAdd(&totals[RenderStats::kMaxBounceStats + k], static_cast<unsigned long long>(queueCounts[kLineWords * (b + 1)]));
    const bool self = ((selfMask >> b) & 1ull) != 0ull;
    if (self)
    {
        const unsigned long long rays = queueCounts[kLineWords * (b + 1)];
        atomicAdd(&totals[3 * RenderStats::kMaxBounceStats + k], rays - shadowListCounts[kLineWords * b]);
        atomicAdd(&counters->shadowRays, rays);
    }
    if ((lookMask >> b) & 1ull)
    {
        const unsigned long long rays = self ? shadowListCounts[kLineWords * b] : queueCounts[kLineWords * (b + 1)], answered = rays - listCounts[kLineWords * b];
        atomicAdd(&totals[2 * RenderStats::kMaxBounceStats + k], answered);
        atomicAdd(&lookBatch[0], answered);
        atomicAdd(&lookBatch[1], rays);
    }
}

__global__ void kTonemap(const float4* image, uint32_t n, uint32_t accumulatedSamples, float exposure, uint32_t* out)
{
    const uint32_t i = blockIdx.x * blockDim.x + threadIdx.x;
    if (i >= n) return;
    const float4 px = image[i];
    const float  in[3] = {px.x, px.y, px.z};
    uint32_t     q[3];
    for (int c = 0; c < 3; ++c)
    {
        const float est = in[c] / static_cast<float>(accumulatedSamples);
        const float x = exposure * est;
        const float a = 2.51f, b = 0.03f, cc = 2.43f, d = 0.59f, e = 0.14f;
        float       y = (x * (a * x + b)) / (x * (cc * x + d) + e);
        y = minf(maxf(y, 0.0f), 1.0f);
        const float srgb = wPow(y, 1.0f / 2.2f);
        q[c] = static_cast<uint32_t>(floorf(srgb * 255.0f + 0.5f));
    }
    out[i] = q[2] | (q[1] << 8) | (q[0] << 16) | (255u << 24);
}

__device__ __forceinline__ Vec3 offsetPositionDeferred(Vec3 p, Vec3 n)
{
    constexpr float kOrigin = 1.0f / 32.0f, kFloatScale = 1.0f / 16384.0f, kIntScale = 1024.0f;
    const int       ox = static_cast<int>(kIntScale * n.x), oy = static_cast<int>(kIntScale * n.y), oz = static_cast<int>(kIntScale * n.z);
    const Vec3      shifted = vec3(__int_as_float(__float_as_int(p.x) + (p.x < 0 ? -ox : ox)), __int_as_float(__float_as_int(p.y) + (p.y < 0 ? -oy : oy)),
                                   __int_as_float(__float_as_int(p.z) + (p.z < 0 ? -oz : oz)));
    return vec3(fabsf(p.x) < kOrigin ? p.x + kFloatScale * n.x : shifted.x, fabsf(p.y) < kOrigin ? p.y + kFloatScale * n.y : shifted.y,
                fabsf(p.z) < kOrigin ? p.z + kFloatScale * n.z : shifted.z);
}

struct DeferredSurface
{
    Vec3 plain, offset, normal, albedo;
};

__device__ __forceinline__ DeferredSurface deferredSurface(const DeviceScene& scene, const float* lut, const ClosestHit& h)
{
    DeferredSurface out;
    const Vec3 p0 = load3(scene.triangles + kTriStride * h.triangle), p1 = load3(scene.triangles + kTriStride * h.triangle + 1),
               p2 = load3(scene.triangles + kTriStride * h.triangle + 2);
    const Vec3 e1 = p1 - p0, e2 = p2 - p0;
    out.plain = p0 + h.u * e1 + h.v * e2;
    out.offset = offsetPositionDeferred(out.plain, normalize(cross(e1, e2)));
    const float4* va = scene.attributes + 4 * static_cast<size_t>(h.triangle);
    const float4  a0 = va[0], a1 = va[1], a2 = va[2], a3 = va[3];
    const Vec3    n0 = vec3(a0.x, a0.y, a0.z), n1 = vec3(a0.w, a1.x, a1.y), n2 = vec3(a1.z, a1.w, a2.x);
    const float   b0 = 1.0f - h.u - h.v, b1 = h.u, b2 = h.v;
    out.normal = (b0 * n0 + b1 * n1) + b2 * n2;
    const float uvx = (b0 * a2.y + b1 * a2.w) + b2 * a3.y, uvy = (b0 * a2.z + b1 * a3.x) + b2 * a3.z;
    out.albedo = evalTexture(scene, lut, __float_as_uint(a3.w), uvx, uvy);
    return out;
}

__device__ __forceinline__ Vec3 skyWithSun(const SkyStateGpu& sky, Vec3 v)
{
    const Vec3  s = vec3(sky.sunDirection[0], sky.sunDirection[1], sky.sunDirection[2]);
    const float theta = wAcos(v.y), gamma = wAcos(minf(maxf(dot(v, s), -1.0f), 1.0f));
    const float cosGamma = wCos(gamma), cosTheta = fabsf(wCos(theta));
    const bool  inDisk = gamma / __uint_as_float(0x3B91D640u) <= 1.0f;
    return vec3(skyRadiance(sky, cosTheta, gamma, cosGamma, 0) + (inDisk ? sky.solarRadiances[0] : 0.0f),
                skyRadiance(sky, cosTheta, gamma, cosGamma, 1) + (inDisk ? sky.solarRadiances[1] : 0.0f),
                skyRadiance(sky, cosTheta, gamma, cosGamma, 2) + (inDisk ? sky.solarRadiances[2] : 0.0f));
}

__global__ __launch_bounds__(kBlock) void kDeferredLighting(DeviceScene scene, SkyStateGpu sky, SunBasis sunBasis, Camera cam, uint32_t width, uint32_t height,
                                                             uint32_t frameCount, float jitterX, float jitterY, float exposure, float* sampleBuffer,
                                                             float* accumulationBuffer, uint32_t* bgraOut, DeviceCounters* counters)
{
    __shared__ uint32_t sStack[kLdsStack * kBlock];
    __shared__ float    sLut[256];
    sLut[threadIdx.x] = scene.albedoLut[threadIdx.x];
    __syncthreads();
    const uint32_t blocksX = (width + 7u) / 8u;
    const uint32_t wave = (blockIdx.x * kBlock + threadIdx.x) >> 6, lane = threadIdx.x & 63u;
    const uint32_t x = (wave % blocksX) * 8u + (lane & 7u), y = (wave / blocksX) * 8u + (lane >> 3);
    unsigned long long closest = 0, shadow = 0;
    if (x < width && y < height)
    {
    const float W = static_cast<float>(width), H = static_cast<float>(height);
    const float su = (static_cast<float>(x) + 0.5f) / W - (jitterX - 0.5f) / (2.0f * W);
    const float tv = (1.0f - (static_cast<float>(y) + 0.5f) / H) - (jitterY - 0.5f) / (2.0f * H);
    const Vec3  rd = normalize(cam.lowerLeftCorner + cam.horizontal * su + cam.vertical * tv - cam.origin);
    TraversalCounters  tc;
    ClosestHit         h;
    closest = 1;
    Vec3               color;
    const Vec3         lightIntensity = vec3(sky.solarRadiances[0], sky.solarRadiances[1], sky.solarRadiances[2]);
    if (!traverse<false, false>(scene, cam.origin, rd, kTMax, &sStack[threadIdx.x], h, tc)) color = skyWithSun(sky, rd);
    else
    {
        DeferredSurface sf = deferredSurface(scene, sLut, h);
        Vec3            normal = sf.normal, albedo = sf.albedo;
        Vec3            position = offsetPositionDeferred(sf.plain, normal);
        float           ux, uy;
        animatedBlueNoise(scene.blueNoise, x, y, frameCount, 1u << 20, ux, uy);
        const float phi = 2.0f * kPi * uy;
        const float cosPhi = wCos(phi), sinPhi = wSin(phi);
        const Vec3  light = sunSample(sky, sunBasis, ux, cosPhi, sinPhi);
        const auto  lightSample = [&](Vec3 pos, Vec3 n, Vec3 alb) {
            const Vec3 reflectance = (alb * kFrac1Pi) * dot(n, light);
            ClosestHit unused;
            ++shadow;
            const float vis = traverse<true, false>(scene, pos, light, kTMax, &sStack[threadIdx.x], unused, tc) ? 0.0f : 1.0f;
            return ((lightIntensity * reflectance) * vis) * __uint_as_float(kSolarInvPdfBits);
        };
        Vec3 radiance = vec3(0.0f, 0.0f, 0.0f), throughput = vec3(1.0f, 1.0f, 1.0f);
        radiance = radiance + throughput * lightSample(position, normal, albedo);
        for (int bounce = 1; bounce < 2; ++bounce)
        {
            const float sinTheta = rf_sqrt(1.0f - ux);
            Vec3        bu, bv;
            pixarOnb(normal, bu, bv);
            const Vec3 wi = basisTimes(bu, bv, normal, vec3(cosPhi * sinTheta, sinPhi * sinTheta, rf_sqrt(ux)));
            throughput = throughput * albedo;
            ++closest;
            if (traverse<false, false>(scene, position, wi, kTMax, &sStack[threadIdx.x], h, tc))
            {
                sf = deferredSurface(scene, sLut, h);
                position = sf.offset;
                normal = sf.normal;
                albedo = sf.albedo;
            }
            else
            {
// ... 55 lines not shown
```

rayfinder_amd/csrc/rf_trace.hip:

```cpp
#include "rf_kernels.hpp"

namespace rf
{
namespace
{
template<bool COUNT>
__global__ __launch_bounds__(kBlock) void kTraceClosest(DeviceScene scene, PathStreams ps, const uint32_t* queue,
                                                         const uint32_t* queueCount, DeviceCounters* counters)
{
    __shared__ uint32_t sStack[kLdsStack * kBlock];
    const uint32_t      i = blockIdx.x * kBlock + threadIdx.x;
    const uint32_t      count = *queueCount;
    if (blockIdx.x * kBlock >= count) return;
    TraversalCounters tc;
    if (i < count)
    {
        const Vec3 o = load3(ps.rayO + i);
        const Vec3 d = load3(ps.rayD + i);
        ClosestHit h;
        traverse<false, COUNT>(scene, o, d, kTMax, &sStack[threadIdx.x], h, tc);
        if (tc.abandoned) atomicAdd(&counters->abandonedRays, 1ull);
        ps.hit[i] = make_float4(__uint_as_float(h.triangle), h.u, h.v, h.t);
    }
    if (COUNT)
// ... 894 lines not shown
            if (node >= kNodeDone) ++phaseLeafIdle;
            else if (static_cast<int32_t>(node) >= 0) ++phaseLeafInterior;
        }
#endif
        bool denseDone = false;
        if constexpr (!COUNT && DENSE_LEAVES)
        {
            const uint32_t     kDenseMin = (flags >> kFlagDenseLeafShift) & 15u;
            constexpr uint32_t kDenseMaxLeaf = 16u;
            const bool         atLeafD = node - kWideLeafBit < kNodeDone - kWideLeafBit;
            if (kDenseMin != 0u && __ballot(atLeafD && ((node >> kWideIndexBits) & 7u) + 1u >= kDenseMin) != 0ull)
            {
                uint32_t firstD = 0u, cnt = 0u, hintD = 0u;
                bool     rejected = false;
                if (atLeafD)
                {
                    firstD = node & ((1u << kWideIndexBits) - 1u), cnt = ((node >> kWideIndexBits) & 7u) + 1u;
                    if (cnt == 8u)
                    {
                        const uint2 big = wide.bigLeaves[firstD];
                        firstD = big.x;
                        cnt = big.y;
                    }
                    if (cnt > kDenseMaxLeaf) cnt = 0u;
                    else if (leafBoxAtLeaf)
                    {
                        const float* t0 = reinterpret_cast<const float*>(scene.triangles + kTriStride * static_cast<size_t>(firstD));
                        const float  loX = t0[3], loY = t0[7], loZ = t0[11];
                        const float4 hi = *reinterpret_cast<const float4*>(t0 + 12);
                        if constexpr (kOccluderCache) hintD = __float_as_uint(hi.w);
                        PackedRay exact = pr;
                        if (kConservative && __builtin_expect((negMask & 8u) != 0u, 0))
                        {
                            const float inf = __uint_as_float(0x7F800000u);
                            if (fabsf(exact.iXY.x) == 1e30f) exact.iXY.x = __builtin_copysignf(inf, exact.iXY.x);
                            if (fabsf(exact.iXY.y) == 1e30f) exact.iXY.y = __builtin_copysignf(inf, exact.iXY.y);
                            if (fabsf(exact.iZ) == 1e30f) exact.iZ = __builtin_copysignf(inf, exact.iZ);
                        }
                        float bn, bf;
                        bool  boxNaN;
                        slabSingleBounds(exact, loX, loY, loZ, hi.x, hi.y, hi.z, bn, bf, boxNaN);
                        if (__builtin_expect((negMask & 8u) != 0u && boxNaN, 0)) cnt = 0u;
                        else if (!(bn <= bf && bf > 0.0f && bn < rayTMax))
                        {
                            cnt = 0u;
                            rejected = true;
                        }
                    }
                }
                bool dealt = rejected;
                bool stopped = false;
                const uint32_t incl = waveScanInclusive<false>(cnt), off = incl - cnt;
                const uint32_t total = static_cast<uint32_t>(__builtin_amdgcn_readlane(static_cast<int>(incl), 63));
                const uint32_t pairTrips = (total + 63u) / 64u;
                const bool     goDense = (pairTrips <= 1u) || (pairTrips <= 2u && __ballot(cnt >= 5u) != 0ull) || (pairTrips <= 4u && __ballot(cnt >= 9u) != 0ull);
                if (goDense)
                {
                    const float oX = pr.oXY.x, oY = pr.oXY.y, oZ = pr.oZ;
                    uint32_t    base = 0u;
                    while (base < total)
                    {
                        const unsigned long long over = __ballot(cnt != 0u && off >= base && off + cnt > base + 64u);
                        const uint32_t           next = over != 0ull ? static_cast<uint32_t>(__builtin_amdgcn_readlane(static_cast<int>(off), __builtin_ctzll(over))) : total;
                        const bool               inTrip = cnt != 0u && off >= base && off < next;
                        const uint32_t           segLo = off - base;
                        const uint32_t           pairs = next - base;
                        const unsigned long long longer = __ballot(inTrip && cnt >= 2u);
                        const uint32_t           dump = (pairs < 64u || longer == 0ull) ? (pairs & 63u) : static_cast<uint32_t>(__builtin_amdgcn_readlane(static_cast<int>(segLo), __builtin_ctzll(longer))) + 1u;
                        const uint32_t           mark = static_cast<uint32_t>(__builtin_amdgcn_ds_permute(static_cast<int>((inTrip ? segLo : dump) << 2), static_cast<int>(inTrip ? lane + 1u : 0u)));
                        const uint32_t           owner = waveScanInclusive<true>(mark) - 1u;
                        const bool               pairLive = lane < pairs;
                        const uint32_t           src = pairLive ? owner : lane;
                        const uint32_t           triOfPair = laneGather(firstD - off, src) + base + lane;
                        const Vec3               po = vec3(laneGather(oX, src), laneGather(oY, src), laneGather(oZ, src));
                        const Vec3               pd = vec3(laneGather(rayDir.x, src), laneGather(rayDir.y, src), laneGather(rayDir.z, src));
                        const float              pTMax = ANY_HIT ? tMax : laneGather(rayTMax, src);
                        TriangleHit              th{};
                        bool                     pairHit = false;
                        if (pairLive)
                        {
                            const v3f a = *reinterpret_cast<const v3f*>(scene.triangles + kTriStride * static_cast<size_t>(triOfPair));
                            const v3f b = *reinterpret_cast<const v3f*>(scene.triangles + kTriStride * static_cast<size_t>(triOfPair) + 1);
                            const v3f c = *reinterpret_cast<const v3f*>(scene.triangles + kTriStride * static_cast<size_t>(triOfPair) + 2);
                            pairHit = intersectTriangle(po, pd, vec3(a.x, a.y, a.z), vec3(b.x, b.y, b.z), vec3(c.x, c.y, c.z), pTMax, th);
                        }
                        const unsigned long long hitMask = __ballot(pairHit);
                        uint32_t                 mine = inTrip ? static_cast<uint32_t>(hitMask >> segLo) & ((1u << cnt) - 1u) : 0u;
                        if constexpr (ANY_HIT)
                        {
                            if (mine != 0u) stopped = true;
                        }
                        else
                        {
                            while (__ballot(mine != 0u) != 0ull)
                            {
                                const uint32_t j = mine != 0u ? static_cast<uint32_t>(__builtin_ctz(mine)) : 0u;
                                const uint32_t from = mine != 0u ? segLo + j : lane;
                                const float    tj = laneGather(th.t, from), uj = laneGather(th.u, from), vj = laneGather(th.v, from);
                                if (mine != 0u && tj < rayTMax)
                                {
                                    rayTMax = tj;
                                    best.u = uj;
                                    best.v = vj;
                                    best.triangle = firstD + j;
                                }
                                mine &= mine - 1u;
                            }
                        }
                        if (inTrip) dealt = true;
                        base = next;
                    }
                }
                else dealt = false;
                if (dealt)
                {
                    if (ANY_HIT && stopped)
                    {
                        occluded = true;
                        if (kOccluderCache) occluderWord = hintD != 0u ? hintD : node;
                        node = kNodeDone;
                    }
                    else popNext();
                }
                denseDone = dealt;
            }
        }
        if (node - kWideLeafBit < kNodeDone - kWideLeafBit && !denseDone)
        {
            uint32_t first = node & ((1u << kWideIndexBits) - 1u), n = ((node >> kWideIndexBits) & 7u) + 1u;
            if (n == 8u)
            {
                const uint2 big = wide.bigLeaves[first];
                first = big.x;
                n = big.y;
            }
            bool finished = false;
            if (kPhase) ++wLeafPhase;
            float4 firstA{}, firstB{}, firstC{};
            uint32_t leafHint = 0u;
            if (leafBoxAtLeaf)
            {
                static_assert(kTriStride * sizeof(float4) == 64, "the leaf phase addresses triangle records by a 32-bit byte offset: 64 bytes each, indices below 2^26");
                const float4* t0 = reinterpret_cast<const float4*>(reinterpret_cast<const char*>(scene.triangles) + (first << 6));
                float4 hi;
                {
                    typedef float v4f __attribute__((ext_vector_type(4)));
                    const v4f* t4 = reinterpret_cast<const v4f*>(t0);
                    v4f        ra = t4[0], rb = t4[1], rc = t4[2];
                    if constexpr (kOccluderCache)
                    {
                        v4f rd = t4[3];
                        asm volatile("" : "+v"(ra), "+v"(rb), "+v"(rc), "+v"(rd));
                        hi = make_float4(rd.x, rd.y, rd.z, rd.w);
                    }
                    else
                    {
                        v3f h3 = *reinterpret_cast<const v3f*>(t0 + 3);
                        asm volatile("" : "+v"(ra), "+v"(rb), "+v"(rc), "+v"(h3));
                        hi = make_float4(h3.x, h3.y, h3.z, 0.0f);
                    }
                    firstA = make_float4(ra.x, ra.y, ra.z, ra.w), firstB = make_float4(rb.x, rb.y, rb.z, rb.w), firstC = make_float4(rc.x, rc.y, rc.z, rc.w);
                }
                if constexpr (kOccluderCache) leafHint = __float_as_uint(hi.w);
                float     bn, bf;
                bool      boxNaN;
                PackedRay exact = pr;
                if (kConservative && __builtin_expect((negMask & 8u) != 0u, 0))
                {
                    const float inf = __uint_as_float(0x7F800000u);
                    if (fabsf(exact.iXY.x) == 1e30f) exact.iXY.x = __builtin_copysignf(inf, exact.iXY.x);
                    if (fabsf(exact.iXY.y) == 1e30f) exact.iXY.y = __builtin_copysignf(inf, exact.iXY.y);
                    if (fabsf(exact.iZ) == 1e30f) exact.iZ = __builtin_copysignf(inf, exact.iZ);
                }
                slabSingleBounds(exact, firstA.w, firstB.w, firstC.w, hi.x, hi.y, hi.z, bn, bf, boxNaN);
                if (__builtin_expect((negMask & 8u) != 0u && boxNaN, 0))
                {
                    needScalar = true;
                    stackSize = spBase, negMask &= 0xFFu;
                    n = 0;
                }
                else if (!(bn <= bf && bf > 0.0f && bn < rayTMax)) n = 0;
            }
            for (uint32_t i = 0; i < n; ++i)
            {
                if (kPhase) ++wLeaf;
                const uint32_t tri = first + i;
                Vec3           p0, p1, p2;
                const uint32_t uTri = __builtin_amdgcn_readfirstlane(tri);
                if (leafBoxAtLeaf && i == 0u)
                {
                    p0 = vec3(firstA.x, firstA.y, firstA.z), p1 = vec3(firstB.x, firstB.y, firstB.z), p2 = vec3(firstC.x, firstC.y, firstC.z);
                }
                else if (uniformTri && __ballot(tri != uTri) == 0ull)
                {
                    typedef uint32_t u8v __attribute__((ext_vector_type(8)));
                    typedef uint32_t u4v __attribute__((ext_vector_type(4)));
                    const float4* ut = scene.triangles + kTriStride * static_cast<size_t>(uTri);
                    u8v           ab;
                    u4v           cc;
                    asm volatile("s_load_dwordx8 %0, %2, 0x0\n\ts_load_dwordx4 %1, %2, 0x20\n\ts_waitcnt lgkmcnt(0)" : "=&s"(ab), "=&s"(cc) : "s"(ut) : "memory");
                    p0 = vec3(__uint_as_float(ab.s0), __uint_as_float(ab.s1), __uint_as_float(ab.s2));
                    p1 = vec3(__uint_as_float(ab.s4), __uint_as_float(ab.s5), __uint_as_float(ab.s6));
                    p2 = vec3(__uint_as_float(cc.x), __uint_as_float(cc.y), __uint_as_float(cc.z));
                }
                else
                {
                    const v3f a = *reinterpret_cast<const v3f*>(scene.triangles + kTriStride * tri);
                    const v3f b = *reinterpret_cast<const v3f*>(scene.triangles + kTriStride * tri + 1);
                    const v3f c = *reinterpret_cast<const v3f*>(scene.triangles + kTriStride * tri + 2);
                    p0 = vec3(a.x, a.y, a.z), p1 = vec3(b.x, b.y, b.z), p2 = vec3(c.x, c.y, c.z);
                }
                if (COUNT) ++rayTris;
#if defined(RF_EXP_PHASE)
                ++phaseTris;
#endif
                TriangleHit th;
                if (intersectTriangle(vec3(pr.oXY.x, pr.oXY.y, pr.oZ), rayDir, p0, p1, p2, rayTMax, th))
                {
                    if (ANY_HIT)
                    {
                        occluded = true;
                        finished = true;
                        break;
                    }
                    rayTMax = th.t;
                    best.u = th.u;
                    best.v = th.v;
                    best.triangle = tri;
                }
            }
            if (finished)
            {
                if (kOccluderCache) occluderWord = leafHint != 0u ? leafHint : node;
#if defined(RF_EXP_PHASE)
                if (ANY_HIT) { ++phaseOccluded; if (phaseFromCache && stackSize == spBase + kSpStep) ++phaseOccHit; }
#endif
                node = kNodeDone;
            }
            else popNext();
        }
        } while (kEagerLeaves && __popcll(__ballot(node - kWideLeafBit < kNodeDone - kWideLeafBit)) >= kLeafRepeat);

        if (kSpill && node == kNodeDone && !needScalar && !occluded)
        {
            while (node == kNodeDone && (negMask >> 8) != 0u)
            {
                unspill();
                popNext();
            }
        }
        if (node == kNodeDone)
        {
            if (needScalar)
            {
                TraversalCounters c2;
                atomicAdd(&counters->scalarRedo[ANY_HIT ? 1 : 0], 1ull);
                best.triangle = kMiss;
                occluded = traverse<ANY_HIT, COUNT, 0>(scene, vec3(pr.oXY.x, pr.oXY.y, pr.oZ), rayDir, tMax, nullptr, best, c2);
                if (c2.abandoned) atomicAdd(&counters->abandonedRays, 1ull);
                rayTMax = best.triangle != kMiss ? best.t : tMax;
                rayNodes = c2.nodesVisited;
                rayTris = c2.triangleTests;
                rayStackHigh = c2.stackHigh;
            }
            if (COUNT)
            {
                tc.nodesVisited += rayNodes;
                tc.triangleTests += rayTris;
                tc.stackHigh = max(tc.stackHigh, rayStackHigh);
            }
            if constexpr (kOccluderCache)
            {
                if (occluderCache && (occluderWord != 0u || (!occluded && (negMask & kNegTriedHint) != 0u)))
                {
                    uint32_t* const cell = wide.occGrid + kOccSlots * static_cast<size_t>(occluderCell(pr.oXY.x, pr.oXY.y, pr.oZ));
                    uint32_t        old[kOccSlots], now[kOccSlots];
                    loadOccluderCell(cell, old);
                    if (occluderWord == 0u)
                    {
#pragma unroll
                        for (int k = 0; k < kOccSlots; ++k) now[k] = k + 1 < kOccSlots ? old[k + 1 < kOccSlots ? k + 1 : k] : 0u;
                        storeOccluderCell(cell, now);
                    }
                    else if (occluderWord != old[0])
                    {
                        int at = kOccSlots - 1;
#pragma unroll
                        for (int k = kOccSlots - 2; k >= 1; --k)
                            if (old[k] == occluderWord) at = k;
                        now[0] = occluderWord;
#pragma unroll
                        for (int k = 1; k < kOccSlots; ++k) now[k] = k <= at ? old[k - 1] : old[k];
                        storeOccluderCell(cell, now);
                    }
                }
            }
            if (ANY_HIT)
            {
                const float visibility = occluded ? 0.0f : 1.0f;
                const Vec3  add = (pendingTerm * visibility) * __uint_as_float(kSolarInvPdfBits);
// ... 14 lines not shown

    if (COUNT)
    {
        const unsigned long long nv = waveSum(tc.nodesVisited), tt = waveSum(tc.triangleTests);
        const uint32_t           sh = waveMax(tc.stackHigh);
        if (lane == 0)
        {
            atomicAdd(ANY_HIT ? &counters->shadowNodeVisits : &counters->closestNodeVisits, nv);
            atomicAdd(ANY_HIT ? &counters->shadowTriangleTests : &counters->closestTriangleTests, tt);
            if (!ANY_HIT) atomicMax(&counters->stackHigh, sh);
        }
        const unsigned long long rf = waveSum(recordFetches);
        if (lane == 0) atomicAdd(ANY_HIT ? &counters->shadowRecordFetches : &counters->closestRecordFetches, rf);
        const int                k = ANY_HIT ? 1 : 0;
        const unsigned long long pops = waveSum(wPop);
        const uint32_t           d = waveMax(wDescend), l = waveMax(wLeaf), lp = waveMax(wLeafPhase), r = waveMax(wRefill), o = waveMax(wOuter);
        if (lane == 0)
        {
            atomicAdd(&counters->descendTrips[k], static_cast<unsigned long long>(d));
            atomicAdd(&counters->leafTrips[k], static_cast<unsigned long long>(l));
            atomicAdd(&counters->leafPhases[k], static_cast<unsigned long long>(lp));
            atomicAdd(&counters->refillTrips[k], static_cast<unsigned long long>(r));
            atomicAdd(&counters->popLaneTrips[k], pops);
            atomicAdd(&counters->outerTrips[k], static_cast<unsigned long long>(o));
        }
    }
#if defined(RF_EXP_PHASE)
    if (!COUNT)
    {
        const int                k = ANY_HIT ? 1 : 0;
        const unsigned long long laneSteps = waveSum(recordFetches), laneLeaves = waveSum(wLeafPhase), laneTris = waveSum(phaseTris);
        const uint32_t           d = waveMax(wDescend), lp = waveMax(phaseLeafWave), r = waveMax(wRefill), o = waveMax(wOuter);
        if (lane == 0)
        {
            atomicAdd(ANY_HIT ? &counters->shadowRecordFetches : &counters->closestRecordFetches, laneSteps);
            atomicAdd(&counters->descendTrips[k], static_cast<unsigned long long>(d));
            atomicAdd(&counters->leafPhases[k], static_cast<unsigned long long>(lp));
            atomicAdd(&counters->leafTrips[k], laneLeaves);
            atomicAdd(&counters->popLaneTrips[k], laneTris);
            atomicAdd(&counters->refillTrips[k], static_cast<unsigned long long>(r));
            atomicAdd(&counters->outerTrips[k], static_cast<unsigned long long>(o));
        }
        const unsigned long long pk = waveSum(phaseParked), pi = waveSum(phaseIdle), li = waveSum(phaseLeafInterior), ld = waveSum(phaseLeafIdle);
        if (lane == 0) atomicAdd(&counters->descendParked[k], pk), atomicAdd(&counters->descendIdle[k], pi), atomicAdd(&counters->leafInterior[k], li), atomicAdd(&counters->leafIdle[k], ld);
        const unsigned long long ot = waveSum(phaseOccTried), oh = waveSum(phaseOccHit), oc = waveSum(phaseOccluded);
        if (lane == 0 && ANY_HIT) atomicAdd(&counters->occluderTried, ot), atomicAdd(&counters->occluderHit, oh), atomicAdd(&counters->occludedRays, oc);
    }
#endif
    if (blockIdx.x == 0 && threadIdx.x == 0 && !(flags & kFlagNoRayCount)) atomicAdd(ANY_HIT ? &counters->shadowRays : &counters->closestRays, static_cast<unsigned long long>(count));
}


__global__ __launch_bounds__(kBlock) void kShadowFirstLook(DeviceScene scene, WideScene wide, SkyStateGpu sky, SunBasis sunBasis, PathStreams ps, const uint32_t* queue,
                                                            const uint32_t* inList, const uint32_t* inCount, uint32_t* list, uint32_t* listCount, DeviceCounters* counters, float tMax,
                                                            uint32_t flags)
{
    __shared__ uint32_t sScratch[8];
    const uint32_t      count = *inCount;
    const uint32_t      firstBounce = flags & kLookFirstBounce;
    const uint32_t      tiles = (count + kItems * kBlock - 1) / (kItems * kBlock);
    if (blockIdx.x == 0 && threadIdx.x == 0 && !(flags & kLookNoRayCount)) atomicAdd(&counters->shadowRays, static_cast<unsigned long long>(count));
    for (uint32_t tile = blockIdx.x; tile < tiles; tile += gridDim.x)
    {
        bool     keep[kItems];
        uint32_t entry[kItems];
#pragma unroll
        for (int k = 0; k < kItems; ++k)
        {
            const uint32_t j = (tile * kItems + k) * kBlock + threadIdx.x;
            keep[k] = j < count;
            entry[k] = j;
            if (j >= count) continue;
            const uint32_t i = inList != nullptr ? inList[j] : j;
            entry[k] = i;
            v3fu           o3 = *reinterpret_cast<const v3fu*>(ps.rayO + i);
            asm volatile("" : "+v"(o3));
            const Vec3     o = vec3(o3.x, o3.y, o3.z);
            uint32_t* const cell = wide.occGrid + kOccSlots * static_cast<size_t>(occluderCellIndex(wide, o.x, o.y, o.z));
            uint32_t        e[kOccSlots];
            loadOccluderCell(cell, e);
            if (e[0] == 0u) continue;
            const Vec3    nz = load3(ps.noiseOut + i);
            const Vec3    dir = sunSample(sky, sunBasis, nz.x, nz.y, nz.z);
            const RayPrep ray = prepareRay(o, dir);
            if (classifyRay(ray) != kRayPlain) continue;
            entry[k] = i | 0x80000000u;
            const PackedRay pr = packRay(ray);
            int             at = -1;
#pragma unroll
            for (int j = 0; j < kOccSlots; ++j)
            {
                const uint32_t w = e[j];
                if (at >= 0 || (w & kWideLeafBit) == 0u || ((w >> kWideIndexBits) & 7u) == 7u) continue;
                const uint32_t first = w & ((1u << kWideIndexBits) - 1u), n = ((w >> kWideIndexBits) & 7u) + 1u;
                const float4*  t0 = scene.triangles + kTriStride * static_cast<size_t>(first);
                typedef float v4f __attribute__((ext_vector_type(4)));
                const v4f*     t4 = reinterpret_cast<const v4f*>(t0);
                v4f            a = t4[0], b = t4[1], c = t4[2];
                v3f            hi = *reinterpret_cast<const v3f*>(t0 + 3);
                asm volatile("" : "+v"(a), "+v"(b), "+v"(c), "+v"(hi));
                float          bn, bf;
                bool           boxNaN;
                slabSingleBounds(pr, a.w, b.w, c.w, hi.x, hi.y, hi.z, bn, bf, boxNaN);
                if (!(bn <= bf && bf > 0.0f && bn < tMax)) continue;
                TriangleHit th;
                bool        stopped = intersectTriangle(o, dir, vec3(a.x, a.y, a.z), vec3(b.x, b.y, b.z), vec3(c.x, c.y, c.z), tMax, th);
                for (uint32_t t = 1; t < n && !stopped; ++t)
                {
                    const v3f q0 = *reinterpret_cast<const v3f*>(t0 + kTriStride * t), q1 = *reinterpret_cast<const v3f*>(t0 + kTriStride * t + 1),
                              q2 = *reinterpret_cast<const v3f*>(t0 + kTriStride * t + 2);
                    stopped = intersectTriangle(o, dir, vec3(q0.x, q0.y, q0.z), vec3(q1.x, q1.y, q1.z), vec3(q2.x, q2.y, q2.z), tMax, th);
                }
                if (stopped) at = j;
            }
            if (at < 0) continue;
            keep[k] = false;
            if (at > 0)
            {
                uint32_t now[kOccSlots];
                now[0] = e[at];
#pragma unroll
                for (int j = 1; j < kOccSlots; ++j) now[j] = j <= at ? e[j - 1] : e[j];
                storeOccluderCell(cell, now);
            }
            const Vec3 add = (load3(ps.pending + i) * 0.0f) * __uint_as_float(kSolarInvPdfBits);
            const bool unchanged = firstBounce == 0u && add.x == 0.0f && add.y == 0.0f && add.z == 0.0f;
            if (!unchanged)
            {
                const uint32_t slot = queue[i];
                const Vec3     radiance = (firstBounce != 0u ? vec3(0.0f, 0.0f, 0.0f) : load3(ps.rad + slot)) + add;
                ps.rad[slot] = make_float4(radiance.x, radiance.y, radiance.z, 0.0f);
            }
        }
        blockAppend<kItems>(keep, entry, list, listCount, sScratch);
    }
}


#if defined(RF_EXP_LEGACY_LAYOUTS)
constexpr int kPacketDepth = 24;

template<bool ANY_HIT>
__global__ __launch_bounds__(kBlock, 6) void kTracePacket(DeviceScene scene, WideScene wide, SkyStateGpu sky, SunBasis sunBasis, PathStreams ps,
                                                          const uint32_t* queue, const uint32_t* queueCount, DeviceCounters* counters, float tMax, uint32_t flags)
{
    __shared__ float    sTMin[kPacketDepth * kBlock];
    const uint32_t      count = *queueCount;
    const uint32_t      lane = __lane_id(), wave = threadIdx.x >> 6;
    const bool          shadowDirFromStream = flags & kFlagShadowDirFromStream;
    const bool          firstBounce = flags & kFlagFirstBounce;
    const float         kInf = __uint_as_float(0x7F800000u);
    float* const        myTMin = sTMin + threadIdx.x;
    const uint32_t      numChunks = (count + 63u) / 64u;
    const uint32_t      totalWaves = gridDim.x * (kBlock / 64);

    for (uint32_t chunkIdx = blockIdx.x * (kBlock / 64) + wave; chunkIdx < numChunks; chunkIdx += totalWaves)
    {
        const uint32_t idx = chunkIdx * 64u + lane;
        const bool     valid = idx < count;
        uint32_t       slot = 0;
        Vec3           o = vec3(0.0f, 0.0f, 0.0f), dir = vec3(0.0f, 0.0f, 1.0f);
        if (valid)
        {
            if (ANY_HIT) slot = loadQ(queue + idx);
            o = load3s(ps.rayO + idx);
            if (ANY_HIT && !shadowDirFromStream)
            {
                const Vec3 nz = load3s(ps.noiseOut + idx);
                dir = sunSample(sky, sunBasis, nz.x, nz.y, nz.z);
            }
            else dir = load3s(ps.rayD + idx);
        }
        const RayPrep   ray = prepareRay(o, dir);
        const PackedRay pr = packRay(ray);
        const uint32_t  rayClass = classifyRay(ray);
        const uint32_t  negMask = ray.negX | (ray.negY << 1) | (ray.negZ << 2);
        bool            needScalar = valid && rayClass != kRayPlain;
        const bool      regular = valid && rayClass == kRayPlain;
        float           rootTMin;
        const bool      rootOk = slabBounds(ray, wide.rootLo, wide.rootHi, rootTMin);
        ClosestHit      best{};
        best.triangle = kMiss;
        float resultT = tMax;
        bool  occluded = false;

        unsigned long long todo = __ballot(regular);
        while (todo != 0ull)
        {
            bool member = regular;
            if (!ANY_HIT)
            {
                const uint32_t leader = static_cast<uint32_t>(__ffsll(static_cast<long long>(todo))) - 1u;
                const uint32_t uNeg = __builtin_amdgcn_readlane(negMask, leader);
                member = regular && ((todo >> lane) & 1ull) != 0ull && negMask == uNeg;
// ... 10 lines not shown
            bool     overflow = false;
            uint32_t wordStack = 0;
            for (;;)
            {
                node = __builtin_amdgcn_readfirstlane(node);
                bool popNow = false;
                if (static_cast<int32_t>(node) >= 0)
                {
                    typedef uint32_t u8v __attribute__((ext_vector_type(8)));
                    typedef uint32_t u4v __attribute__((ext_vector_type(4)));
                    typedef uint32_t u2v __attribute__((ext_vector_type(2)));
                    const float4* un = wide.nodes + 4 * static_cast<size_t>(node);
                    u8v           a;
                    u4v           b;
                    u2v           c;
                    asm volatile("s_load_dwordx8 %0, %3, 0x0\n\ts_load_dwordx4 %1, %3, 0x20\n\ts_load_dwordx2 %2, %3, 0x30\n\ts_waitcnt lgkmcnt(0)"
                                 : "=&s"(a), "=&s"(b), "=&s"(c)
                                 : "s"(un)
                                 : "memory");
                    const float4   q0 = make_float4(__uint_as_float(a.s0), __uint_as_float(a.s1), __uint_as_float(a.s2), __uint_as_float(a.s3));
                    const float4   q1 = make_float4(__uint_as_float(a.s4), __uint_as_float(a.s5), __uint_as_float(a.s6), __uint_as_float(a.s7));
                    const float4   q2 = make_float4(__uint_as_float(b.x), __uint_as_float(b.y), __uint_as_float(b.z), __uint_as_float(b.w));
                    const uint32_t axis = (c.x >> kWideAxisShift) & 3u;
                    const uint32_t word0 = c.x & ~(3u << kWideAxisShift), word1 = c.y;
                    float          t0, t1;
                    bool           ok0, ok1;
                    slabPair(pr, q0, q1, q2, ok0, t0, ok1, t1);
                    const bool hit0 = active && ok0 && t0 < limit, hit1 = active && ok1 && t1 < limit;
                    const unsigned long long m0 = __ballot(hit0), m1 = __ballot(hit1);
                    bool secondFirst;
                    if (ANY_HIT) secondFirst = 2 * __popcll(__ballot(hit0 && hit1 && t1 < t0)) > __popcll(m0 & m1);
                    else secondFirst = ((passNeg >> axis) & 1u) != 0u;
                    const unsigned long long mN = secondFirst ? m1 : m0, mF = secondFirst ? m0 : m1;
                    const uint32_t           nearWord = secondFirst ? word1 : word0, farWord = secondFirst ? word0 : word1;
                    const bool               hitN = secondFirst ? hit1 : hit0, hitF = secondFirst ? hit0 : hit1;
                    const float              tF = secondFirst ? t0 : t1;
                    if (mN != 0ull)
                    {
                        if (mF != 0ull)
                        {
                            if (depth >= kPacketDepth)
                            {
                                overflow = true;
                                break;
                            }
                            myTMin[depth * kBlock] = hitF ? tF : kInf;
                            {
                                uint32_t keepM0;
                                asm volatile("s_mov_b32 %1, m0\n\ts_mov_b32 m0, %3\n\ts_nop 0\n\tv_writelane_b32 %0, %2, m0\n\ts_mov_b32 m0, %1"
                                             : "+v"(wordStack), "=&s"(keepM0)
                                             : "s"(farWord), "s"(depth));
                            }
                            ++depth;
                        }
                        node = nearWord;
                        active = hitN;
                    }
                    else if (mF != 0ull)
                    {
                        node = farWord;
                        active = hitF;
                    }
                    else popNow = true;
                }
                else
                {
                    uint32_t first = node & ((1u << kWideIndexBits) - 1u), n = ((node >> kWideIndexBits) & 7u) + 1u;
                    if (n == 8u)
                    {
                        const uint2 big = wide.bigLeaves[first];
                        first = __builtin_amdgcn_readfirstlane(big.x);
                        n = __builtin_amdgcn_readfirstlane(big.y);
                    }
                    for (uint32_t i = 0; i < n; ++i)
                    {
                        typedef uint32_t u8v __attribute__((ext_vector_type(8)));
                        typedef uint32_t u4v __attribute__((ext_vector_type(4)));
                        const uint32_t tri = first + i;
                        const float4*  ut = scene.triangles + kTriStride * static_cast<size_t>(tri);
                        u8v            ab;
                        u4v            cc;
                        asm volatile("s_load_dwordx8 %0, %2, 0x0\n\ts_load_dwordx4 %1, %2, 0x20\n\ts_waitcnt lgkmcnt(0)" : "=&s"(ab), "=&s"(cc) : "s"(ut) : "memory");
                        const Vec3 p0 = vec3(__uint_as_float(ab.s0), __uint_as_float(ab.s1), __uint_as_float(ab.s2));
                        const Vec3 p1 = vec3(__uint_as_float(ab.s4), __uint_as_float(ab.s5), __uint_as_float(ab.s6));
                        const Vec3 p2 = vec3(__uint_as_float(cc.x), __uint_as_float(cc.y), __uint_as_float(cc.z));
                        TriangleHit th;
                        if (active && intersectTriangle(o, dir, p0, p1, p2, limit, th))
                        {
                            if (ANY_HIT)
                            {
                                occluded = true;
                                limit = -kInf;
                                active = false;
                            }
                            else
                            {
                                limit = th.t;
                                best.u = th.u;
                                best.v = th.v;
                                best.triangle = tri;
                            }
                        }
                    }
                    if (ANY_HIT && __ballot(member && !occluded) == 0ull) break;
                    popNow = true;
                }
                if (popNow)
                {
                    bool found = false;
                    while (depth > 0)
                    {
                        --depth;
                        const float tm = myTMin[depth * kBlock];
                        active = tm < limit;
                        if (__ballot(active) != 0ull)
                        {
                            node = __builtin_amdgcn_readlane(wordStack, static_cast<uint32_t>(depth));
                            found = true;
                            break;
                        }
                    }
                    if (!found) break;
                }
            }
            if (overflow)
            {
                if (member)
                {
                    needScalar = true;
                    best.triangle = kMiss;
                    occluded = false;
                }
            }
            else if (member) resultT = limit;
        }

        if (needScalar)
        {
            TraversalCounters c2;
            atomicAdd(&counters->scalarRedo[ANY_HIT ? 1 : 0], 1ull);
            best.triangle = kMiss;
            occluded = traverse<ANY_HIT, false, 0>(scene, o, dir, tMax, nullptr, best, c2);
            if (c2.abandoned) atomicAdd(&counters->abandonedRays, 1ull);
            resultT = best.triangle != kMiss ? best.t : tMax;
        }
        if (valid)
        {
            if (ANY_HIT)
            {
                const float visibility = occluded ? 0.0f : 1.0f;
                const Vec3  add = (load3s(ps.pending + idx) * visibility) * __uint_as_float(kSolarInvPdfBits);
                const Vec3  radiance = (firstBounce ? vec3(0.0f, 0.0f, 0.0f) : load3s(ps.rad + slot)) + add;
                store4s(ps.rad + slot, radiance.x, radiance.y, radiance.z, 0.0f);
            }
            else store4s(ps.hit + idx, __uint_as_float(best.triangle), best.u, best.v, resultT);
        }
    }
    if (blockIdx.x == 0 && threadIdx.x == 0) atomicAdd(ANY_HIT ? &counters->shadowRays : &counters->closestRays, static_cast<unsigned long long>(count));
}
#endif

__global__ void kHitPoints(DeviceScene scene, const float4* hit, P3* rayO, uint32_t n)
{
    const uint32_t i = blockIdx.x * blockDim.x + threadIdx.x;
    if (i >= n) return;
    const float4   h = hit[i];
    const uint32_t tri = __float_as_uint(h.x);
    if (tri == kMiss) return;
    const Vec3 hp = hitPoint(scene, tri, h.y, h.z);
    store3(rayO + i, hp);
}

__global__ __launch_bounds__(kBlock) void kPrimaryStats(DeviceScene scene, Camera cam, uint32_t width, uint32_t height,
                                                         uint32_t* nodesVisited, uint8_t* hitOut, float* tOut, uint32_t* triTests, DeviceCounters* counters)
{
    __shared__ uint32_t sStack[kLdsStack * kBlock];
    const uint32_t blocksX = (width + 7u) / 8u;
    const uint32_t wave = (blockIdx.x * kBlock + threadIdx.x) >> 6;
    const uint32_t lane = threadIdx.x & 63u;
    const uint32_t j = (wave % blocksX) * 8u + (lane & 7u);
    const uint32_t i = (wave / blocksX) * 8u + (lane >> 3);
    if (j >= width || i >= height) return;
    const float u = static_cast<float>(j) / static_cast<float>(width);
    const float v = 1.0f - static_cast<float>(i + 1) / static_cast<float>(height);
    const Vec3  dir = normalize(cam.lowerLeftCorner + cam.horizontal * u + cam.vertical * v - cam.origin);
    ClosestHit        h;
    TraversalCounters tc;
    const bool        found = traverse<false, true>(scene, cam.origin, dir, FLT_MAX, &sStack[threadIdx.x], h, tc);
    if (tc.abandoned) atomicAdd(&counters->abandonedRays, 1ull);
    const size_t      k = static_cast<size_t>(i) * width + j;
    nodesVisited[k] = tc.nodesVisited;
    if (hitOut) hitOut[k] = found ? 1 : 0;
    if (tOut) tOut[k] = found ? h.t : 0.0f;
    if (triTests) triTests[k] = tc.triangleTests;
}

__global__ __launch_bounds__(kBlock) void kIntersectRays(DeviceScene scene, const float* rays, uint64_t n, float tMax, uint32_t* triOut,
                                                          float* tOut, float* uvOut, float* pOut, uint32_t* nvOut, uint32_t* ttOut, DeviceCounters* counters)
{
    __shared__ uint32_t sStack[kLdsStack * kBlock];
    const uint64_t      i = static_cast<uint64_t>(blockIdx.x) * kBlock + threadIdx.x;
    if (i >= n) return;
    const float*      r = rays + 6 * i;
    ClosestHit        h;
    TraversalCounters tc;
    const bool        found = traverse<false, true>(scene, vec3(r[0], r[1], r[2]), vec3(r[3], r[4], r[5]), tMax, &sStack[threadIdx.x], h, tc);
    if (tc.abandoned) atomicAdd(&counters->abandonedRays, 1ull);
    triOut[i] = h.triangle;
    if (tOut) tOut[i] = found ? h.t : 0.0f;
    if (uvOut)
    {
        uvOut[2 * i] = found ? h.u : 0.0f;
        uvOut[2 * i + 1] = found ? h.v : 0.0f;
    }
    if (pOut)
    {
        pOut[3 * i] = found ? h.p.x : 0.0f;
        pOut[3 * i + 1] = found ? h.p.y : 0.0f;
        pOut[3 * i + 2] = found ? h.p.z : 0.0f;
    }
    if (nvOut) nvOut[i] = tc.nodesVisited;
    if (ttOut) ttOut[i] = tc.triangleTests;
}

__global__ __launch_bounds__(kBlock) void kOccludedRays(DeviceScene scene, const float* rays, uint64_t n, float tMax, float* visOut, DeviceCounters* counters)
{
    __shared__ uint32_t sStack[kLdsStack * kBlock];
    const uint64_t      i = static_cast<uint64_t>(blockIdx.x) * kBlock + threadIdx.x;
    if (i >= n) return;
    const float*      r = rays + 6 * i;
    ClosestHit        h;
    TraversalCounters tc;
    const bool        occluded = traverse<true, false>(scene, vec3(r[0], r[1], r[2]), vec3(r[3], r[4], r[5]), tMax, &sStack[threadIdx.x], h, tc);
    if (tc.abandoned) atomicAdd(&counters->abandonedRays, 1ull);
    visOut[i] = occluded ? 0.0f : 1.0f;
}


}

namespace kern
{
TraceWideKernel traceWideKernel(bool anyHit, bool count, bool nearestFirst, int compact, bool denseLeaves)
{
#define RF_TW(A, C, N, L, D) \
    if (anyHit == A && count == C && nearestFirst == N && compact == L && denseLeaves == D) return kTraceWide<A, C, N, L, D>;
    RF_TW(false, true, false, 0, false) RF_TW(true, true, true, 0, false) RF_TW(true, true, false, 0, false)
    RF_TW(false, false, false, 0, false) RF_TW(false, false, false, 3, false) RF_TW(false, false, false, 4, false) RF_TW(false, false, false, 5, false) RF_TW(false, false, false, 6, false)
    RF_TW(false, false, false, 3, true) RF_TW(false, false, false, 4, true) RF_TW(false, false, false, 5, true)
    RF_TW(true, false, true, 0, false) RF_TW(true, false, false, 0, false)
    RF_TW(true, false, true, 3, false) RF_TW(true, false, false, 3, false) RF_TW(true, false, true, 4, false) RF_TW(true, false, false, 4, false) RF_TW(true, false, true, 5, false) RF_TW(true, false, false, 5, false)
    RF_TW(true, false, true, 3, true) RF_TW(true, false, false, 4, true) RF_TW(true, false, false, 5, true)
#if defined(RF_EXP_LEGACY_LAYOUTS)
    RF_TW(false, false, false, 1, false) RF_TW(false, false, false, 2, false) RF_TW(true, false, true, 1, false) RF_TW(true, false, true, 2, false)
#endif
#undef RF_TW
    return nullptr;
}
TraceClosestKernel    traceClosestKernel(bool count) { return count ? kTraceClosest<true> : kTraceClosest<false>; }
TraceShadowKernel     traceShadowKernel(bool count) { return count ? kTraceShadow<true> : kTraceShadow<false>; }
ShadowFirstLookKernel shadowFirstLookKernel() { return kShadowFirstLook; }
TracePacketKernel     tracePacketKernel(bool anyHit)
{
#if defined(RF_EXP_LEGACY_LAYOUTS)
    return anyHit ? kTracePacket<true> : kTracePacket<false>;
#else
    (void)anyHit;
    return nullptr;
#endif
}
HitPointsKernel     hitPointsKernel() { return kHitPoints; }
PrimaryStatsKernel  primaryStatsKernel() { return kPrimaryStats; }
IntersectRaysKernel intersectRaysKernel() { return kIntersectRays; }
OccludedRaysKernel  occludedRaysKernel() { return kOccludedRays; }
}
}
```

Baseline: 12960.

## Precompute triangle edges at upload and use refined fast reciprocal in ray prep

Triangles are rewritten on the device after upload so that the second and third vertices hold edge vectors e1 and e2. This removes two vector subtractions per triangle test and per hit-point reconstruction. Ray and determinant reciprocals now use a hardware rcp with one Newton refinement step, guarded by a wave-uniform ballot that falls back to IEEE division for extreme operands. A self-test API checks bit-exactness of the fast reciprocal over all floats. The scheme relies on every triangle consumer being updated to the edge layout, and it adds register-pinning asm barriers.

```diff
diff --git a/include/rayfinder_amd.h b/include/rayfinder_amd.h
--- a/include/rayfinder_amd.h
+++ b/include/rayfinder_amd.h
@@ -198,6 +198,8 @@
 RF_API int rf_renderer_bind_accumulation_buffer(rf_renderer* r, void* device_ptr, uint64_t bytes);
 
 RF_API int rf_device_count(int32_t* count_out);
+RF_API int rf_selftest_reciprocal(int32_t device_ordinal, uint64_t* mismatches, uint32_t* first_mismatch, uint64_t* fast_operands, const uint32_t* probes,
+                                  uint32_t num_probes, uint8_t* probe_fast);
 typedef struct rf_comm rf_comm;
 #define RF_COMM_ID_BYTES 128
 #define RF_GATHER_LOOPBACK 1u
diff --git a/rayfinder_amd/__init__.py b/rayfinder_amd/__init__.py
--- a/rayfinder_amd/__init__.py
+++ b/rayfinder_amd/__init__.py
@@ -363,6 +363,15 @@
     return n.value
 
 
+def selftest_reciprocal(probes=(), device_ordinal=0):
+    p = np.ascontiguousarray(np.asarray(probes, np.uint32).reshape(-1))
+    fast = np.zeros(p.size, np.uint8)
+    bad, first, nfast = C.c_uint64(0), C.c_uint32(0), C.c_uint64(0)
+    check(lib.rf_selftest_reciprocal(device_ordinal, C.byref(bad), C.byref(first), C.byref(nfast), _ptr(p) if p.size else None, p.size, _ptr(fast) if p.size else None))
+    return dict(mismatches=int(bad.value), first_mismatch=None if first.value == 0xFFFFFFFF and bad.value == 0 else int(first.value), fast_operands=int(nfast.value),
+                probe_fast=fast.astype(bool))
+
+
 def comm_unique_id():
     buf = np.zeros(128, np.uint8)
     check(lib.rf_comm_unique_id(_ptr(buf)))
diff --git a/rayfinder_amd/_ffi.py b/rayfinder_amd/_ffi.py
--- a/rayfinder_amd/_ffi.py
+++ b/rayfinder_amd/_ffi.py
@@ -169,6 +169,7 @@
     "rf_renderer_accumulation_device_buffer": (C.c_int, [C.c_void_p, C.POINTER(C.c_void_p), C.POINTER(C.c_uint64)]),
     "rf_renderer_bind_accumulation_buffer": (C.c_int, [C.c_void_p, C.c_void_p, C.c_uint64]),
     "rf_device_count": (C.c_int, [C.POINTER(C.c_int32)]),
+    "rf_selftest_reciprocal": (C.c_int, [C.c_int32, C.POINTER(C.c_uint64), C.POINTER(C.c_uint32), C.POINTER(C.c_uint64), C.c_void_p, C.c_uint32, C.c_void_p]),
     "rf_comm_unique_id": (C.c_int, [C.c_void_p]),
     "rf_comm_create": (C.c_int, [C.c_void_p, C.c_uint32, C.c_uint32, C.c_int32, C.POINTER(C.c_void_p)]),
     "rf_comm_destroy": (None, [C.c_void_p]),
diff --git a/rayfinder_amd/csrc/rf_c_api.cpp b/rayfinder_amd/csrc/rf_c_api.cpp
--- a/rayfinder_amd/csrc/rf_c_api.cpp
+++ b/rayfinder_amd/csrc/rf_c_api.cpp
@@ -722,6 +722,18 @@
     return guarded([&] {
         require(count_out, "null argument");
         *count_out = rf::deviceCount();
+        return RF_OK;
+    });
+}
+
+int rf_selftest_reciprocal(int32_t device_ordinal, uint64_t* mismatches, uint32_t* first_mismatch, uint64_t* fast_operands, const uint32_t* probes, uint32_t num_probes,
+                           uint8_t* probe_fast)
+{
+    return guarded([&] {
+        require(mismatches && first_mismatch && fast_operands, "null argument");
+        require(num_probes == 0 || (probes && probe_fast), "null argument");
+        require(num_probes <= 65536u, "too many probes");
+        rf::selftestReciprocal(device_ordinal, probes, num_probes, *mismatches, *first_mismatch, *fast_operands, probe_fast);
         return RF_OK;
     });
 }
diff --git a/rayfinder_amd/csrc/rf_device.hpp b/rayfinder_amd/csrc/rf_device.hpp
--- a/rayfinder_amd/csrc/rf_device.hpp
+++ b/rayfinder_amd/csrc/rf_device.hpp
@@ -35,12 +35,64 @@
     uint32_t negX, negY, negZ;
 };
 
+constexpr float kRcpFastLo = 1e-30f, kRcpFastHi = 1e30f;
+__device__ __forceinline__ bool rcpFast(float x)
+{
+    const float a = fabsf(x);
+    return a >= kRcpFastLo && a <= kRcpFastHi;
+}
+__device__ __forceinline__ float rcpRefined(float x)
+{
+    const float y = __builtin_amdgcn_rcpf(x);
+    const float e = __builtin_fmaf(-x, y, 1.0f);
+    return __builtin_fmaf(e, y, y);
+}
+__device__ __forceinline__ float rcpIeee(float x)
+{
+    asm volatile("" : "+v"(x));
+    return 1.0f / x;
+}
+__device__ __forceinline__ float rfRcp(float x)
+{
+#if defined(RF_EXP_RCP_IEEE)
+    return 1.0f / x;
+#elif defined(RF_EXP_RCP_DIVERGENT)
+    if (__builtin_expect(rcpFast(x), 1)) return rcpRefined(x);
+    return rcpIeee(x);
+#else
+    if (__builtin_expect(__ballot(!rcpFast(x)) == 0ull, 1)) return rcpRefined(x);
+    return rcpIeee(x);
+#endif
+}
+
+__device__ __forceinline__ float rfRcpAbove(float x)
+{
+#if defined(RF_EXP_RCP_IEEE)
+    return 1.0f / x;
+#elif defined(RF_EXP_RCP_DIVERGENT)
+    if (__builtin_expect(fabsf(x) <= kRcpFastHi, 1)) return rcpRefined(x);
+    return rcpIeee(x);
+#else
+    if (__builtin_expect(__ballot(!(fabsf(x) <= kRcpFastHi)) == 0ull, 1)) return rcpRefined(x);
+    return rcpIeee(x);
+#endif
+}
+
+template<bool FAST_RCP = true>
 __device__ __forceinline__ RayPrep prepareRay(Vec3 o, Vec3 d)
 {
     RayPrep r;
     r.origin = o;
     r.direction = d;
-    r.invDir = vec3(1.0f / d.x, 1.0f / d.y, 1.0f / d.z);
+#if defined(RF_EXP_RCP_IEEE) || defined(RF_EXP_RCP_DIVERGENT)
+    r.invDir = vec3(rfRcp(d.x), rfRcp(d.y), rfRcp(d.z));
+    (void)FAST_RCP;
+#else
+    if constexpr (!FAST_RCP) r.invDir = vec3(1.0f / d.x, 1.0f / d.y, 1.0f / d.z);
+    else
+    if (__builtin_expect(__ballot(!(rcpFast(d.x) && rcpFast(d.y) && rcpFast(d.z))) == 0ull, 1)) r.invDir = vec3(rcpRefined(d.x), rcpRefined(d.y), rcpRefined(d.z));
+    else r.invDir = vec3(rcpIeee(d.x), rcpIeee(d.y), rcpIeee(d.z));
+#endif
     r.negX = r.invDir.x < 0.0f;
     r.negY = r.invDir.y < 0.0f;
     r.negZ = r.invDir.z < 0.0f;
@@ -85,17 +137,17 @@
     float t, u, v;
 };
 
+template<bool PIN_S = false, bool FAST_RCP = true>
 __device__ __forceinline__ bool
-intersectTriangle(Vec3 origin, Vec3 direction, Vec3 p0, Vec3 p1, Vec3 p2, float rayTMax, TriangleHit& hit)
+intersectTriangle(Vec3 origin, Vec3 direction, Vec3 p0, Vec3 e1, Vec3 e2, float rayTMax, TriangleHit& hit)
 {
     constexpr float kEpsilon = 0.00001f;
-    const Vec3      e1 = p1 - p0;
-    const Vec3      e2 = p2 - p0;
     const Vec3      h = cross(direction, e2);
     const float     det = dot(e1, h);
     if (det > -kEpsilon && det < kEpsilon) return false;
-    const float invDet = 1.0f / det;
-    const Vec3  s = origin - p0;
+    const float invDet = FAST_RCP ? rfRcpAbove(det) : 1.0f / det;
+    Vec3        s = origin - p0;
+    if constexpr (PIN_S) asm volatile("" : "+v"(s.x), "+v"(s.y), "+v"(s.z));
     const float u = invDet * dot(s, h);
     if (u < 0.0f || u > 1.0f) return false;
     const Vec3  q = cross(s, e1);
@@ -111,11 +163,23 @@
     }
     return false;
 }
+template<bool PIN_S = false>
 __device__ __forceinline__ bool
-intersectTriangle(const RayPrep& r, Vec3 p0, Vec3 p1, Vec3 p2, float rayTMax, TriangleHit& hit)
-{
-    return intersectTriangle(r.origin, r.direction, p0, p1, p2, rayTMax, hit);
-}
+intersectTriangle(const RayPrep& r, Vec3 p0, Vec3 e1, Vec3 e2, float rayTMax, TriangleHit& hit)
+{
+    return intersectTriangle<PIN_S>(r.origin, r.direction, p0, e1, e2, rayTMax, hit);
+}
+template<bool FAST_RCP = true>
+__device__ __forceinline__ bool
+intersectTriangleVertices(Vec3 origin, Vec3 direction, Vec3 p0, Vec3 p1, Vec3 p2, float rayTMax, TriangleHit& hit)
+{
+    return intersectTriangle<false, FAST_RCP>(origin, direction, p0, p1 - p0, p2 - p0, rayTMax, hit);
+}
+#if defined(RF_EXP_SHADE_FAST_RCP)
+constexpr bool kMemoryBoundFastRcp = true;
+#else
+constexpr bool kMemoryBoundFastRcp = false;
+#endif
 
 struct ClosestHit
 {
@@ -166,13 +230,12 @@
                     const float4   c = scene.triangles[kTriStride * tri + 2];
                     if (COUNT) ++counters.triangleTests;
                     TriangleHit th;
-                    const Vec3  p0 = vec3(a.x, a.y, a.z), p1 = vec3(b.x, b.y, b.z), p2 = vec3(c.x, c.y, c.z);
-                    if (intersectTriangle(ray, p0, p1, p2, rayTMax, th))
+                    const Vec3  p0 = vec3(a.x, a.y, a.z), e1 = vec3(b.x, b.y, b.z), e2 = vec3(c.x, c.y, c.z);
+                    if (intersectTriangle<true>(ray, p0, e1, e2, rayTMax, th))
                     {
                         if (ANY_HIT) return true;
                         rayTMax = th.t;
                         found = true;
-                        const Vec3 e1 = p1 - p0, e2 = p2 - p0;
                         const Vec3 p = p0 + th.u * e1 + th.v * e2;
                         const Vec3 n = normalize(cross(e1, e2));
                         out.p = offsetRay(p, n);
diff --git a/rayfinder_amd/csrc/rf_kernels.hpp b/rayfinder_amd/csrc/rf_kernels.hpp
--- a/rayfinder_amd/csrc/rf_kernels.hpp
+++ b/rayfinder_amd/csrc/rf_kernels.hpp
@@ -263,9 +263,8 @@
 
 __device__ __forceinline__ Vec3 hitPoint(const DeviceScene& scene, uint32_t tri, float u, float v)
 {
-    const Vec3 p0 = load3(scene.triangles + kTriStride * tri), p1 = load3(scene.triangles + kTriStride * tri + 1),
-               p2 = load3(scene.triangles + kTriStride * tri + 2);
-    const Vec3   e1 = p1 - p0, e2 = p2 - p0;
+    const Vec3 p0 = load3(scene.triangles + kTriStride * tri), e1 = load3(scene.triangles + kTriStride * tri + 1),
+               e2 = load3(scene.triangles + kTriStride * tri + 2);
     const Vec3   p = p0 + u * e1 + v * e2;
     return offsetRay(p, normalize(cross(e1, e2)));
 }
@@ -328,6 +327,7 @@
 using ShadowFirstLookKernel = void (*)(DeviceScene scene, WideScene wide, SkyStateGpu sky, SunBasis sunBasis, PathStreams ps, const uint32_t* queue, const uint32_t* inList, const uint32_t* inCount, uint32_t* list, uint32_t* listCount, DeviceCounters* counters, float tMax, uint32_t flags);
 using TracePacketKernel = void (*)(DeviceScene scene, WideScene wide, SkyStateGpu sky, SunBasis sunBasis, PathStreams ps, const uint32_t* queue, const uint32_t* queueCount, DeviceCounters* counters, float tMax, uint32_t flags);
 using HitPointsKernel = void (*)(DeviceScene scene, const float4* hit, P3* rayO, uint32_t n);
+using TriangleEdgesKernel = void (*)(float4* triangles, uint64_t n);
 using BounceTotalsKernel = void (*)(const uint32_t* queueCounts, uint32_t numBounces, unsigned long long* totals, const uint32_t* listCounts, unsigned long long lookMask, unsigned long long* lookBatch, const uint32_t* shadowListCounts, unsigned long long selfMask, DeviceCounters* counters);
 using TonemapKernel = void (*)(const float4* image, uint32_t n, uint32_t accumulatedSamples, float exposure, uint32_t* out);
 using PrimaryStatsKernel = void (*)(DeviceScene scene, Camera cam, uint32_t width, uint32_t height, uint32_t* nodesVisited, uint8_t* hitOut, float* tOut, uint32_t* triTests, DeviceCounters* counters);
@@ -341,6 +341,7 @@
 ShadowFirstLookKernel shadowFirstLookKernel();
 TracePacketKernel     tracePacketKernel(bool anyHit);
 HitPointsKernel       hitPointsKernel();
+TriangleEdgesKernel   triangleEdgesKernel();
 PrimaryStatsKernel    primaryStatsKernel();
 IntersectRaysKernel   intersectRaysKernel();
 OccludedRaysKernel    occludedRaysKernel();
diff --git a/rayfinder_amd/csrc/rf_renderer.hip b/rayfinder_amd/csrc/rf_renderer.hip
--- a/rayfinder_amd/csrc/rf_renderer.hip
+++ b/rayfinder_amd/csrc/rf_renderer.hip
@@ -1228,6 +1228,12 @@
             m.optQuadHalfFromBounce = m.optQuadHalfShadowFromBounce = m.optQuadLocalFromBounce = m.optQuadLocalShadowFromBounce = m.optOctFromBounce = 0u;
         }
         m.triangles.upload(padded.data(), padded.size());
+        if (n)
+        {
+            hipLaunchKernelGGL(triangleEdgesKernel(), dim3(static_cast<uint32_t>((n + 255) / 256)), dim3(256), 0, m.stream, m.triangles.ptr, static_cast<uint64_t>(n));
+            RF_HIP(hipGetLastError());
+            RF_HIP(hipStreamSynchronize(m.stream));
+        }
     }
     {
         const size_t        n = sceneView.vertexAttributes.size();
diff --git a/rayfinder_amd/csrc/rf_renderer.hpp b/rayfinder_amd/csrc/rf_renderer.hpp
--- a/rayfinder_amd/csrc/rf_renderer.hpp
+++ b/rayfinder_amd/csrc/rf_renderer.hpp
@@ -273,4 +273,6 @@
 };
 
 uint32_t checkWideLayouts(std::span<const BvhNode> nodes, float* quadHalfAreaRatio = nullptr);
+
+void selftestReciprocal(int deviceOrdinal, const uint32_t* probes, uint32_t numProbes, uint64_t& mismatches, uint32_t& firstMismatch, uint64_t& fastOperands, uint8_t* probeFast);
 }
diff --git a/rayfinder_amd/csrc/rf_shade.hip b/rayfinder_amd/csrc/rf_shade.hip
--- a/rayfinder_amd/csrc/rf_shade.hip
+++ b/rayfinder_amd/csrc/rf_shade.hip
@@ -322,7 +322,7 @@
         bool       settled = false;
         if (selfShadow && cur.boxHi.w != 0.0f)
         {
-            const RayPrep ray = prepareRay(shadowOrigin, lightDirection);
+            const RayPrep ray = prepareRay<kMemoryBoundFastRcp>(shadowOrigin, lightDirection);
             if (classifyRay(ray) == kRayPlain)
             {
                 const PackedRay pr = packRay(ray);
@@ -332,7 +332,7 @@
                 if (bn <= bf && bf > 0.0f && bn < kTMax)
                 {
                     TriangleHit th;
-                    settled = intersectTriangle(shadowOrigin, lightDirection, cur.p0, cur.p1, cur.p2, kTMax, th);
+                    settled = intersectTriangleVertices<kMemoryBoundFastRcp>(shadowOrigin, lightDirection, cur.p0, cur.p1, cur.p2, kTMax, th);
                 }
             }
         }
@@ -490,9 +490,8 @@
 __device__ __forceinline__ DeferredSurface deferredSurface(const DeviceScene& scene, const float* lut, const ClosestHit& h)
 {
     DeferredSurface out;
-    const Vec3 p0 = load3(scene.triangles + kTriStride * h.triangle), p1 = load3(scene.triangles + kTriStride * h.triangle + 1),
-               p2 = load3(scene.triangles + kTriStride * h.triangle + 2);
-    const Vec3 e1 = p1 - p0, e2 = p2 - p0;
+    const Vec3 p0 = load3(scene.triangles + kTriStride * h.triangle), e1 = load3(scene.triangles + kTriStride * h.triangle + 1),
+               e2 = load3(scene.triangles + kTriStride * h.triangle + 2);
     out.plain = p0 + h.u * e1 + h.v * e2;
     out.offset = offsetPositionDeferred(out.plain, normalize(cross(e1, e2)));
     const float4* va = scene.attributes + 4 * static_cast<size_t>(h.triangle);
diff --git a/rayfinder_amd/csrc/rf_trace.hip b/rayfinder_amd/csrc/rf_trace.hip
--- a/rayfinder_amd/csrc/rf_trace.hip
+++ b/rayfinder_amd/csrc/rf_trace.hip
@@ -1000,7 +1000,7 @@
                             const v3f a = *reinterpret_cast<const v3f*>(scene.triangles + kTriStride * static_cast<size_t>(triOfPair));
                             const v3f b = *reinterpret_cast<const v3f*>(scene.triangles + kTriStride * static_cast<size_t>(triOfPair) + 1);
                             const v3f c = *reinterpret_cast<const v3f*>(scene.triangles + kTriStride * static_cast<size_t>(triOfPair) + 2);
-                            pairHit = intersectTriangle(po, pd, vec3(a.x, a.y, a.z), vec3(b.x, b.y, b.z), vec3(c.x, c.y, c.z), pTMax, th);
+                            pairHit = intersectTriangle<true>(po, pd, vec3(a.x, a.y, a.z), vec3(b.x, b.y, b.z), vec3(c.x, c.y, c.z), pTMax, th);
                         }
                         const unsigned long long hitMask = __ballot(pairHit);
                         uint32_t                 mine = inTrip ? static_cast<uint32_t>(hitMask >> segLo) & ((1u << cnt) - 1u) : 0u;
@@ -1103,11 +1103,11 @@
             {
                 if (kPhase) ++wLeaf;
                 const uint32_t tri = first + i;
-                Vec3           p0, p1, p2;
+                Vec3           p0, e1, e2;
                 const uint32_t uTri = __builtin_amdgcn_readfirstlane(tri);
                 if (leafBoxAtLeaf && i == 0u)
                 {
-                    p0 = vec3(firstA.x, firstA.y, firstA.z), p1 = vec3(firstB.x, firstB.y, firstB.z), p2 = vec3(firstC.x, firstC.y, firstC.z);
+                    p0 = vec3(firstA.x, firstA.y, firstA.z), e1 = vec3(firstB.x, firstB.y, firstB.z), e2 = vec3(firstC.x, firstC.y, firstC.z);
                 }
                 else if (uniformTri && __ballot(tri != uTri) == 0ull)
                 {
@@ -1118,22 +1118,23 @@
                     u4v           cc;
                     asm volatile("s_load_dwordx8 %0, %2, 0x0\n\ts_load_dwordx4 %1, %2, 0x20\n\ts_waitcnt lgkmcnt(0)" : "=&s"(ab), "=&s"(cc) : "s"(ut) : "memory");
                     p0 = vec3(__uint_as_float(ab.s0), __uint_as_float(ab.s1), __uint_as_float(ab.s2));
-                    p1 = vec3(__uint_as_float(ab.s4), __uint_as_float(ab.s5), __uint_as_float(ab.s6));
-                    p2 = vec3(__uint_as_float(cc.x), __uint_as_float(cc.y), __uint_as_float(cc.z));
+                    e1 = vec3(__uint_as_float(ab.s4), __uint_as_float(ab.s5), __uint_as_float(ab.s6));
+                    e2 = vec3(__uint_as_float(cc.x), __uint_as_float(cc.y), __uint_as_float(cc.z));
                 }
                 else
                 {
-                    const v3f a = *reinterpret_cast<const v3f*>(scene.triangles + kTriStride * tri);
-                    const v3f b = *reinterpret_cast<const v3f*>(scene.triangles + kTriStride * tri + 1);
-                    const v3f c = *reinterpret_cast<const v3f*>(scene.triangles + kTriStride * tri + 2);
-                    p0 = vec3(a.x, a.y, a.z), p1 = vec3(b.x, b.y, b.z), p2 = vec3(c.x, c.y, c.z);
+                    v3f a = *reinterpret_cast<const v3f*>(scene.triangles + kTriStride * tri);
+                    v3f b = *reinterpret_cast<const v3f*>(scene.triangles + kTriStride * tri + 1);
+                    v3f c = *reinterpret_cast<const v3f*>(scene.triangles + kTriStride * tri + 2);
+                    asm volatile("" : "+v"(a), "+v"(b), "+v"(c));
+                    p0 = vec3(a.x, a.y, a.z), e1 = vec3(b.x, b.y, b.z), e2 = vec3(c.x, c.y, c.z);
                 }
                 if (COUNT) ++rayTris;
 #if defined(RF_EXP_PHASE)
                 ++phaseTris;
 #endif
                 TriangleHit th;
-                if (intersectTriangle(vec3(pr.oXY.x, pr.oXY.y, pr.oZ), rayDir, p0, p1, p2, rayTMax, th))
+                if (intersectTriangle<true>(vec3(pr.oXY.x, pr.oXY.y, pr.oZ), rayDir, p0, e1, e2, rayTMax, th))
                 {
                     if (ANY_HIT)
                     {
@@ -1314,7 +1315,7 @@
             if (e[0] == 0u) continue;
             const Vec3    nz = load3(ps.noiseOut + i);
             const Vec3    dir = sunSample(sky, sunBasis, nz.x, nz.y, nz.z);
-            const RayPrep ray = prepareRay(o, dir);
+            const RayPrep ray = prepareRay<kMemoryBoundFastRcp>(o, dir);
             if (classifyRay(ray) != kRayPlain) continue;
             entry[k] = i | 0x80000000u;
             const PackedRay pr = packRay(ray);
@@ -1336,12 +1337,12 @@
                 slabSingleBounds(pr, a.w, b.w, c.w, hi.x, hi.y, hi.z, bn, bf, boxNaN);
                 if (!(bn <= bf && bf > 0.0f && bn < tMax)) continue;
                 TriangleHit th;
-                bool        stopped = intersectTriangle(o, dir, vec3(a.x, a.y, a.z), vec3(b.x, b.y, b.z), vec3(c.x, c.y, c.z), tMax, th);
+                bool        stopped = intersectTriangle<false, kMemoryBoundFastRcp>(o, dir, vec3(a.x, a.y, a.z), vec3(b.x, b.y, b.z), vec3(c.x, c.y, c.z), tMax, th);
                 for (uint32_t t = 1; t < n && !stopped; ++t)
                 {
                     const v3f q0 = *reinterpret_cast<const v3f*>(t0 + kTriStride * t), q1 = *reinterpret_cast<const v3f*>(t0 + kTriStride * t + 1),
                               q2 = *reinterpret_cast<const v3f*>(t0 + kTriStride * t + 2);
-                    stopped = intersectTriangle(o, dir, vec3(q0.x, q0.y, q0.z), vec3(q1.x, q1.y, q1.z), vec3(q2.x, q2.y, q2.z), tMax, th);
+                    stopped = intersectTriangle<false, kMemoryBoundFastRcp>(o, dir, vec3(q0.x, q0.y, q0.z), vec3(q1.x, q1.y, q1.z), vec3(q2.x, q2.y, q2.z), tMax, th);
                 }
                 if (stopped) at = j;
             }
@@ -1518,10 +1519,10 @@
                         u4v            cc;
                         asm volatile("s_load_dwordx8 %0, %2, 0x0\n\ts_load_dwordx4 %1, %2, 0x20\n\ts_waitcnt lgkmcnt(0)" : "=&s"(ab), "=&s"(cc) : "s"(ut) : "memory");
                         const Vec3 p0 = vec3(__uint_as_float(ab.s0), __uint_as_float(ab.s1), __uint_as_float(ab.s2));
-                        const Vec3 p1 = vec3(__uint_as_float(ab.s4), __uint_as_float(ab.s5), __uint_as_float(ab.s6));
-                        const Vec3 p2 = vec3(__uint_as_float(cc.x), __uint_as_float(cc.y), __uint_as_float(cc.z));
+                        const Vec3 e1 = vec3(__uint_as_float(ab.s4), __uint_as_float(ab.s5), __uint_as_float(ab.s6));
+                        const Vec3 e2 = vec3(__uint_as_float(cc.x), __uint_as_float(cc.y), __uint_as_float(cc.z));
                         TriangleHit th;
-                        if (active && intersectTriangle(o, dir, p0, p1, p2, limit, th))
+                        if (active && intersectTriangle(o, dir, p0, e1, e2, limit, th))
                         {
                             if (ANY_HIT)
                             {
@@ -1672,7 +1673,87 @@
     visOut[i] = occluded ? 0.0f : 1.0f;
 }
 
-
+__global__ void kTriangleEdges(float4* triangles, uint64_t n)
+{
+    const uint64_t i = static_cast<uint64_t>(blockIdx.x) * blockDim.x + threadIdx.x;
+    if (i >= n) return;
+    float4* const t = triangles + kTriStride * i;
+    const float4  a = t[0];
+    float4        b = t[1], c = t[2];
+    b.x = b.x - a.x, b.y = b.y - a.y, b.z = b.z - a.z;
+    c.x = c.x - a.x, c.y = c.y - a.y, c.z = c.z - a.z;
+    t[1] = b;
+    t[2] = c;
+}
+
+__global__ __launch_bounds__(kBlock) void kSelftestReciprocal(unsigned long long* out, uint32_t* first, const uint32_t* probes, uint32_t numProbes, uint8_t* probeFast)
+{
+    const uint64_t     tid = static_cast<uint64_t>(blockIdx.x) * kBlock + threadIdx.x, stride = static_cast<uint64_t>(gridDim.x) * kBlock;
+    if (tid < numProbes) probeFast[tid] = rcpFast(__uint_as_float(probes[tid])) ? 1 : 0;
+    unsigned long long bad = 0, fast = 0;
+    for (uint64_t i = tid; i < (1ull << 32); i += stride)
+    {
+        const uint32_t bits = static_cast<uint32_t>(i);
+        float          x = __uint_as_float(bits);
+        asm volatile("" : "+v"(x));
+        const float got = rcpFast(x) ? rcpRefined(x) : rfRcp(x);
+        float       x4 = x;
+        asm volatile("" : "+v"(x4));
+        const float viaBranch = rfRcp(x4);
+        float       x2 = x;
+        asm volatile("" : "+v"(x2));
+        const float want = 1.0f / x2;
+        bool        same = (__float_as_uint(got) == __float_as_uint(want) || (got != got && want != want)) &&
+                           (__float_as_uint(viaBranch) == __float_as_uint(want) || (viaBranch != viaBranch && want != want));
+        if (!(fabsf(x) < 0.00001f))
+        {
+            float x3 = x;
+            asm volatile("" : "+v"(x3));
+            const float above = rfRcpAbove(x3);
+            same = same && (__float_as_uint(above) == __float_as_uint(want) || (above != above && want != want));
+        }
+        if (!same)
+        {
+            ++bad;
+            atomicMin(first, bits);
+        }
+        if (rcpFast(x)) ++fast;
+    }
+    bad = waveSum(bad), fast = waveSum(fast);
+    if (__lane_id() == 0)
+    {
+        if (bad) atomicAdd(&out[0], bad);
+        atomicAdd(&out[1], fast);
+    }
+}
+
+}
+
+void selftestReciprocal(int deviceOrdinal, const uint32_t* probes, uint32_t numProbes, uint64_t& mismatches, uint32_t& firstMismatch, uint64_t& fastOperands, uint8_t* probeFast)
+{
+    requireDevice(deviceOrdinal);
+    ScopedStream                     stream;
+    DeviceBuffer<unsigned long long> out;
+    DeviceBuffer<uint32_t>           first, dProbes;
+    DeviceBuffer<uint8_t>            dFast;
+    ScopedStream::Drain              drain{stream};
+    const unsigned long long         zero[2] = {0ull, 0ull};
+    const uint32_t                   none = 0xFFFFFFFFu;
+    out.upload(zero, 2);
+    first.upload(&none, 1);
+    dProbes.upload(probes, numProbes);
+    dFast.alloc(numProbes);
+    constexpr uint32_t kGrid = 8192;
+    if (numProbes > kGrid * static_cast<uint32_t>(kBlock)) throw std::invalid_argument("selftestReciprocal: too many probes");
+    hipLaunchKernelGGL(kSelftestReciprocal, dim3(kGrid), dim3(kBlock), 0, stream.handle, out.ptr, first.ptr, dProbes.ptr, numProbes, dFast.ptr);
+    RF_HIP(hipGetLastError());
+    RF_HIP(hipStreamSynchronize(stream.handle));
+    unsigned long long h[2];
+    RF_HIP(hipMemcpy(h, out.ptr, sizeof(h), hipMemcpyDeviceToHost));
+    RF_HIP(hipMemcpy(&firstMismatch, first.ptr, sizeof(uint32_t), hipMemcpyDeviceToHost));
+    if (numProbes) RF_HIP(hipMemcpy(probeFast, dFast.ptr, numProbes, hipMemcpyDeviceToHost));
+    mismatches = h[0];
+    fastOperands = h[1];
 }
 
 namespace kern
@@ -1706,6 +1787,7 @@
 #endif
 }
 HitPointsKernel     hitPointsKernel() { return kHitPoints; }
+TriangleEdgesKernel triangleEdgesKernel() { return kTriangleEdges; }
 PrimaryStatsKernel  primaryStatsKernel() { return kPrimaryStats; }
 IntersectRaysKernel intersectRaysKernel() { return kIntersectRays; }
 OccludedRaysKernel  occludedRaysKernel() { return kOccludedRays; }
```

Result: no change. 13010 (median of 6 runs) (+0.4%).
